# ivannz/cplxmodule

Measured on AMD Instinct MI355X. Metric: Cplx-samples/sec fwd+bwd (CplxLinear-4096 + VD), higher is better.
Workload: dtype bf16; 1 GPU; CplxLinearVD 4096->4096, bf16 activations / fp32 master weights, batch 8192 per GPU, LRT fwd + KL + full bwd (BASELINE configs[1] + VD); global_batch=8192, parallelism=dp1, noise=in-kernel Philox4x32-7, launch=hipGraph replay, warmup_detail=5 eager steps (capture prerequisites) + 5 untimed replays

## Files before the change

### cplxmodule_amd/csrc/gemm.h

```cpp
#pragma once
#include "common.h"
#include "launch.h"

namespace cplxamd {

struct GemmArgs {
  const void* a_r; const void* a_i; int64_t a_rs, a_cs;
  const void* b_r; const void* b_i; int64_t b_rs, b_cs;
  const float* bias_r; const float* bias_i; const float* emul;
  void* c_r; void* c_i; int64_t ldc;
  int M, N, K;
  int conj_b, accumulate;
  int order = 1, group_m = 4, lds_epilogue = 1;
  int splits = 1; int kchunk = 0; void* ws = nullptr; int64_t ws_bytes = 0;
  const float* g1 = nullptr; const float* g2 = nullptr; float gsign = 1.0f;
  int batch = 1; int64_t a_bs = 0, b_bs = 0, c_bs = 0;
  const float* beta = nullptr; int emul_exp = 0;
  int emul_both = 0;
  const void* fx_r = nullptr; const void* fx_i = nullptr; const void* fga = nullptr; int64_t fld = 0;
  const float* scale_a = nullptr; const float* scale_b = nullptr;
  int flags = 0;
  int* plan = nullptr; int ncu = 0;
};

__device__ __forceinline__ float gemm_beta(const GemmArgs& g) { return (g.accumulate && g.beta) ? *g.beta : 1.0f; }
__device__ __forceinline__ float gemm_alpha(const GemmArgs& g) { return g.scale_a ? g.scale_a[1] * g.scale_b[1] : 1.0f; }
__device__ __forceinline__ float gemm_alpha_inv(const GemmArgs& g) { return g.scale_a ? g.scale_a[0] * g.scale_b[0] : 1.0f; }

__device__ __forceinline__ float gemm_emul(const GemmArgs& g, float m) { return g.emul_exp ? expf(m) : m; }

template <bool CPLX>
int launch_gemm_generic(const GemmArgs& g, int in_dtype, int out_dtype, hipStream_t st);

int64_t gemm_generic_ws_bytes(int M, int N, int K, bool cplx);

template <bool CPLX>
int launch_gemm_bf16(const GemmArgs& g, int out_dtype, hipStream_t st);

int launch_gemm_bf16_w4(const GemmArgs& g, bool cplx, int out_dtype, bool ta, bool tb, hipStream_t st, bool& taken);

int launch_gemm_bf16_gauss(const GemmArgs& g, int out_dtype, hipStream_t st);
int64_t gemm_bf16_gauss_ws_bytes(int M, int N, int K);


int64_t gemm_bf16_ws_bytes(int M, int N, int K, bool cplx);

template <bool CPLX>
int launch_gemm_f16(const GemmArgs& g, int out_dtype, hipStream_t st);
int launch_gemm_f16_w4(const GemmArgs& g, bool cplx, int out_dtype, bool ta, bool tb, hipStream_t st, bool& taken);

}
```

### cplxmodule_amd/csrc/gemm_bf16_impl.h

```cpp
#include <type_traits>

#include "gemm.h"
#include "prims.h"

namespace cplxamd {

constexpr int BK = 32, STAGES = 3;
template <bool CPLX>
struct Cfg {
  static constexpr int NT = 512;
  static constexpr int IB = CPLX ? 2 : 4;
  static constexpr int JB = 2;
  static constexpr int WM = CPLX ? 4 : 2, WN = CPLX ? 2 : 4;
  static constexpr int BM = 32 * IB * WM, BN = 32 * JB * WN;
  static constexpr int A_BYTES = BM * BK * 2, B_BYTES = BN * BK * 2;
  static constexpr int STAGE_BYTES = (CPLX ? 2 : 1) * (A_BYTES + B_BYTES);
  static constexpr int SMEM = STAGES * STAGE_BYTES;
  static constexpr int PA = BM * 4 / NT, PB = BN * 4 / NT;
  static constexpr int LOADS = (CPLX ? 2 : 1) * (PA + PB);
};


template <int ROWS, bool T, int NT>
__device__ __forceinline__ uint32_t piece_voff(int64_t ld, int row0, int rows, int j) {
  const int p = j * NT + (int)threadIdx.x;
  if (!T) {
    const int row = p >> 2;
    const int kc = (p & 3) ^ ((row >> 2) & 3);
    int grow = row0 + row;
    grow = grow < rows ? grow : rows - 1;
    return (uint32_t)(((int64_t)(grow - row0) * ld + kc * 8) * 2);
  }
  constexpr int CPR = ROWS / 8;
  const int k = p / CPR;
  const int c = (p % CPR) ^ ((k & 3) << 2);
  int col = row0 + c * 8;
  col = col + 8 <= rows ? col : rows - 8;
  return (uint32_t)(((int64_t)k * ld + (col - row0)) * 2);
}
template <bool T>
__device__ __forceinline__ const bf16_t* piece_base(const bf16_t* plane, int64_t ld, int row0, int k0) {
  return T ? plane + (int64_t)k0 * ld + row0 : plane + (int64_t)row0 * ld + (int64_t)k0;
}

__device__ __forceinline__ bf16x8 frag_n(const char* lds_plane, int row, int kc) {
  const int off = row * 64 + ((kc ^ ((row >> 2) & 3)) << 4);
  return *reinterpret_cast<const bf16x8*>(lds_plane + off);
}

template <int ROWS>
__device__ __forceinline__ bf16x8 frag_t(const char* lds_plane, int rb, int kb, int m) {
  const int r = rb + 4 * (m & 3);
  s16x4 v[2];
#pragma unroll
  for (int h = 0; h < 2; ++h) {
    const int k = kb + 4 * h + (m >> 2);
    const int off = k * (ROWS * 2) + (((r >> 3) ^ ((k & 3) << 2)) << 4) + (r & 7) * 2;
    v[h] = __builtin_amdgcn_ds_read_tr16_b64_v4i16(
        (__attribute__((address_space(3))) s16x4*)(lds_plane + off));
  }
  const s16x8 both = __builtin_shufflevector(v[0], v[1], 0, 1, 2, 3, 4, 5, 6, 7);
  return __builtin_bit_cast(bf16x8, both);
}

__device__ __forceinline__ void nt_store16(void* p, uint4 v) { *reinterpret_cast<uint4*>(p) = v; }
__device__ __forceinline__ void nt_store16(float* p, const f4& a) { st4(p, a); }

template <typename TOUT, bool CPLX, bool CONJ, bool TA, bool TB>
__global__ __launch_bounds__((Cfg<CPLX>::NT), 2) void gemm_bf16_kernel(GemmArgs g) {
  extern __shared__ __attribute__((aligned(16))) char smem[];
  using C = Cfg<CPLX>;
  constexpr int NT = C::NT;

  constexpr int BM = C::BM, BN = C::BN, IB = C::IB, JB = C::JB;
  const int tiles_m = (g.M + BM - 1) / BM, tiles_n = (g.N + BN - 1) / BN;
  const int ntiles = tiles_m * tiles_n;
  int lin = blockIdx.x, split = 0;
  if (g.splits > 1) { split = lin / ntiles; lin -= split * ntiles; }
  int bm, bn;
  if (g.order == 0) {
    bm = lin / tiles_n; bn = lin - bm * tiles_n;
  } else {
    const int q = ntiles >> 3, r = ntiles & 7, xcd = lin & 7, idx = lin >> 3;
    lin = (xcd < r ? xcd * (q + 1) : r * (q + 1) + (xcd - r) * q) + idx;
    const int GM = g.group_m;
    const int per_group = GM * tiles_n;
    const int grp = lin / per_group, in_grp = lin - grp * per_group;
    const int first_m = grp * GM;
    const int gm = (tiles_m - first_m) < GM ? (tiles_m - first_m) : GM;
    bm = first_m + in_grp % gm; bn = in_grp / gm;
  }
  const int m0 = __builtin_amdgcn_readfirstlane(bm * BM), n0 = __builtin_amdgcn_readfirstlane(bn * BN);

  const int lane = threadIdx.x & 63, wid = threadIdx.x >> 6;
  const int wm = (wid / C::WN) * (32 * IB), wn = (wid % C::WN) * (32 * JB);
  const int l31 = lane & 31, lk = lane >> 5;
  const int l15 = lane & 15, lg = (lane >> 4) & 1;

  const bf16_t* Ar = (const bf16_t*)g.a_r; const bf16_t* Ai = (const bf16_t*)g.a_i;
  const bf16_t* Br = (const bf16_t*)g.b_r; const bf16_t* Bi = (const bf16_t*)g.b_i;
  const int64_t lda = TA ? g.a_cs : g.a_rs, ldb = TB ? g.b_cs : g.b_rs;

  f32x16 acc_r[IB][JB], acc_i[CPLX ? IB : 1][JB];
#pragma unroll
  for (int i = 0; i < IB; ++i)
#pragma unroll
    for (int j = 0; j < JB; ++j) {
      acc_r[i][j] = f32x16{0};
      if (CPLX) acc_i[i][j] = f32x16{0};
    }

  const bool bias_in_acc = g.bias_r != nullptr && g.g1 == nullptr && g.splits <= 1;
  f4 bias_v[CPLX ? 2 : 1][JB][4];
  if (bias_in_acc) {
    const bool vec = (g.N & 3) == 0 && (reinterpret_cast<uintptr_t>(g.bias_r) & 15) == 0 &&
                     (!CPLX || (reinterpret_cast<uintptr_t>(g.bias_i) & 15) == 0);
#pragma unroll
    for (int pl = 0; pl < (CPLX ? 2 : 1); ++pl) {
      const float* bias = pl ? g.bias_i : g.bias_r;
#pragma unroll
      for (int j = 0; j < JB; ++j)
#pragma unroll
        for (int q = 0; q < 4; ++q) {
          const int col = n0 + wn + j * 32 + 8 * q + 4 * lk;
          if (vec && col + 3 < g.N) {
            bias_v[pl][j][q] = ld4(bias + col);
          } else {
#pragma unroll
            for (int e = 0; e < 4; ++e) bias_v[pl][j][q].v[e] = col + e < g.N ? bias[col + e] : 0.f;
          }
        }
    }
#ifdef CPLXAMD_GEMM_F16
    if (g.scale_a) {
      const float inv = gemm_alpha_inv(g);
#pragma unroll
      for (int pl = 0; pl < (CPLX ? 2 : 1); ++pl)
#pragma unroll
        for (int j = 0; j < JB; ++j)
#pragma unroll
          for (int q = 0; q < 4; ++q)
#pragma unroll
            for (int e = 0; e < 4; ++e) bias_v[pl][j][q].v[e] *= inv;
    }
#endif
  }
  auto apply_bias = [&]() __attribute__((always_inline)) {
    if (!bias_in_acc) return;
#pragma unroll
    for (int i = 0; i < IB; ++i)
#pragma unroll
      for (int j = 0; j < JB; ++j)
#pragma unroll
        for (int q = 0; q < 4; ++q)
#pragma unroll
          for (int e = 0; e < 4; ++e) {
            acc_r[i][j][4 * q + e] = bias_v[0][j][q].v[e];
            if (CPLX) acc_i[i][j][4 * q + e] = bias_v[CPLX ? 1 : 0][j][q].v[e];
          }
  };
  const int kbase = __builtin_amdgcn_readfirstlane(split * g.kchunk);
  const uint32_t smem_off = lds_offset_of(smem);
  const uint32_t wave_lds = (uint32_t)__builtin_amdgcn_readfirstlane(threadIdx.x >> 6) * 1024u;
  uint32_t voa[C::PA], vob[C::PB];
#pragma unroll
  for (int j = 0; j < C::PA; ++j) voa[j] = piece_voff<BM, TA, NT>(lda, m0, g.M, j);
#pragma unroll
  for (int j = 0; j < C::PB; ++j) vob[j] = piece_voff<BN, TB, NT>(ldb, n0, g.N, j);
  auto stage_q = [&](int buf, int k0, int q) __attribute__((always_inline)) {
    k0 += kbase;
    const uint32_t s = smem_off + (uint32_t)(buf * C::STAGE_BYTES) + wave_lds;
    if (q < C::PA)
      lds_dma16_sv(piece_base<TA>(Ar, lda, m0, k0), voa[q], s + q * NT * 16);
    else if (q < C::PA + C::PB)
      lds_dma16_sv(piece_base<TB>(Br, ldb, n0, k0), vob[q - C::PA], s + C::A_BYTES + (q - C::PA) * NT * 16);
    else if (q < 2 * C::PA + C::PB)
      lds_dma16_sv(piece_base<TA>(Ai, lda, m0, k0), voa[q - C::PA - C::PB],
                   s + C::A_BYTES + C::B_BYTES + (q - C::PA - C::PB) * NT * 16);
    else
      lds_dma16_sv(piece_base<TB>(Bi, ldb, n0, k0), vob[q - 2 * C::PA - C::PB],
                   s + 2 * C::A_BYTES + C::B_BYTES + (q - 2 * C::PA - C::PB) * NT * 16);
  };
  auto stage_all = [&](int buf, int k0) __attribute__((always_inline)) {
#pragma unroll
    for (int q = 0; q < C::LOADS; ++q) stage_q(buf, k0, q);
  };

  auto a_frag = [&](const char* plane, int i, int ks) __attribute__((always_inline)) -> bf16x8 {
    if (TA) return frag_t<BM>(plane, wm + i * 32 + 16 * lg, ks * 16 + 8 * lk, l15);
    return frag_n(plane, wm + i * 32 + l31, ks * 2 + lk);
  };
  auto b_frag = [&](const char* plane, int j, int ks) __attribute__((always_inline)) -> bf16x8 {
    if (TB) return frag_t<BN>(plane, wn + j * 32 + 16 * lg, ks * 16 + 8 * lk, l15);
    return frag_n(plane, wn + j * 32 + l31, ks * 2 + lk);
  };

  const int klen = g.splits > 1 ? ((g.K - kbase) < g.kchunk ? (g.K - kbase) : g.kchunk) : g.K;
  const int nt = __builtin_amdgcn_readfirstlane(klen / BK);
  {
    bf16x8 ar[2][IB], br[2][JB], ai[2][IB], bi[2][JB];
    auto read_half = [&](int buf, int ks) __attribute__((always_inline)) {
      const char* sA = smem + buf * C::STAGE_BYTES;
      const char* sB = sA + C::A_BYTES;
      const char* sAi = sB + C::B_BYTES;
      const char* sBi = sAi + C::A_BYTES;
#pragma unroll
      for (int i = 0; i < IB; ++i) {
        ar[ks][i] = a_frag(sA, i, ks);
        if (CPLX) ai[ks][i] = a_frag(sAi, i, ks);
      }
#pragma unroll
      for (int j = 0; j < JB; ++j) {
        br[ks][j] = b_frag(sB, j, ks);
        if (CPLX) bi[ks][j] = b_frag(sBi, j, ks);
      }
    };
    constexpr int NFRAG = CPLX ? 2 * IB + 4 : IB + JB;
    auto read_one = [&](int buf, int ks, int idx) __attribute__((always_inline)) {
      const char* sA = smem + buf * C::STAGE_BYTES;
      const char* sB = sA + C::A_BYTES;
      const char* sAi = sB + C::B_BYTES;
      const char* sBi = sAi + C::A_BYTES;
      if (CPLX) {
        if (idx == 0) br[ks][0] = b_frag(sB, 0, ks);
        else if (idx == 1) bi[ks][0] = b_frag(sBi, 0, ks);
        else if (idx == 2) ar[ks][0] = a_frag(sA, 0, ks);
        else if (idx == 3) ai[ks][0] = a_frag(sAi, 0, ks);
        else if (idx == 4) br[ks][1] = b_frag(sB, 1, ks);
        else if (idx == 5) bi[ks][1] = b_frag(sBi, 1, ks);
        else if ((idx & 1) == 0) ar[ks][(idx - 4) / 2] = a_frag(sA, (idx - 4) / 2, ks);
        else ai[ks][(idx - 5) / 2] = a_frag(sAi, (idx - 5) / 2, ks);
      } else {
        if (idx == 0) br[ks][0] = b_frag(sB, 0, ks);
        else if (idx == 1) ar[ks][0] = a_frag(sA, 0, ks);
        else if (idx == 2) br[ks][1] = b_frag(sB, 1, ks);
        else if (idx == 3) ar[ks][1] = a_frag(sA, 1, ks);
        else if (idx < 2 + JB) br[ks][idx - 2] = b_frag(sB, idx - 2, ks);
        else ar[ks][idx - JB] = a_frag(sA, idx - JB, ks);
      }
    };
    constexpr int H = (C::LOADS + 1) / 2;
    auto mfma_half = [&](int ks, int slot, int tile, int q0, int q1, int rbuf, int rks) __attribute__((always_inline)) {
      bf16x8 nai[IB];
      if (CPLX) {
#pragma unroll
        for (int i = 0; i < IB; ++i) nai[i] = neg_frag(CONJ ? ar[ks][i] : ai[ks][i]);
      }
      int q = q0;
      const int k0s = (tile < nt ? tile : nt - 1) * BK;
      if constexpr (CPLX) {
        constexpr int NG = 2 * IB * JB;
#pragma unroll
        for (int ph = 0; ph < 2; ++ph)
#pragma unroll
          for (int i = 0; i < IB; ++i)
#pragma unroll
            for (int j = 0; j < JB; ++j) {
              if (ph == 0) {
                acc_r[i][j] = CPLXAMD_MFMA16(br[ks][j], ar[ks][i], acc_r[i][j]);
                acc_i[i][j] = CPLXAMD_MFMA16(br[ks][j], ai[ks][i], acc_i[i][j]);
              } else if (CONJ) {
                acc_r[i][j] = CPLXAMD_MFMA16(bi[ks][j], ai[ks][i], acc_r[i][j]);
                acc_i[i][j] = CPLXAMD_MFMA16(bi[ks][j], nai[i], acc_i[i][j]);
              } else {
                acc_r[i][j] = CPLXAMD_MFMA16(bi[ks][j], nai[i], acc_r[i][j]);
                acc_i[i][j] = CPLXAMD_MFMA16(bi[ks][j], ar[ks][i], acc_i[i][j]);
              }
              constexpr int PER = (NFRAG + NG - 1) / NG;
              const int g0 = (ph * IB * JB + i * JB + j) * PER;
              __builtin_amdgcn_sched_barrier(0);
#pragma unroll
              for (int r = 0; r < PER; ++r)
                if (g0 + r < NFRAG) read_one(rbuf, rks, g0 + r);
              __builtin_amdgcn_sched_barrier(0);
              if (q < q1) {
                __builtin_amdgcn_sched_barrier(0);
                stage_q(slot, k0s, q);
                __builtin_amdgcn_sched_barrier(0);
                ++q;
              }
            }
        return;
      }
#pragma unroll
      for (int i = 0; i < IB; ++i)
#pragma unroll
        for (int j = 0; j < JB; ++j) {
          acc_r[i][j] = CPLXAMD_MFMA16(br[ks][j], ar[ks][i], acc_r[i][j]);
          if (CPLX) {
            acc_i[i][j] = CPLXAMD_MFMA16(br[ks][j], ai[ks][i], acc_i[i][j]);
            if (CONJ) {
              acc_r[i][j] = CPLXAMD_MFMA16(bi[ks][j], ai[ks][i], acc_r[i][j]);
              acc_i[i][j] = CPLXAMD_MFMA16(bi[ks][j], nai[i], acc_i[i][j]);
            } else {
              acc_r[i][j] = CPLXAMD_MFMA16(bi[ks][j], nai[i], acc_r[i][j]);
              acc_i[i][j] = CPLXAMD_MFMA16(bi[ks][j], ar[ks][i], acc_i[i][j]);
            }
          }
          {
            constexpr int PER = (NFRAG + IB * JB - 1) / (IB * JB);
            const int g0 = (i * JB + j) * PER;
            __builtin_amdgcn_sched_barrier(0);
#pragma unroll
            for (int r = 0; r < PER; ++r)
              if (g0 + r < NFRAG) read_one(rbuf, rks, g0 + r);
            __builtin_amdgcn_sched_barrier(0);
          }
          if (q < q1) {
            __builtin_amdgcn_sched_barrier(0);
            stage_q(slot, k0s, q);
            __builtin_amdgcn_sched_barrier(0);
            ++q;
          }
        }
    };
    stage_all(0, 0);
    if (nt > 1) stage_all(1, BK);
    apply_bias();
    if (nt > 1) wait_vmcnt<C::LOADS>(); else wait_vmcnt<0>();
    __builtin_amdgcn_s_barrier();
    read_half(0, 0);
#pragma unroll
    for (int q = 0; q < H; ++q) stage_q(2, (nt > 2 ? 2 : nt - 1) * BK, q);
    auto tile_body = [&](int cur, int nx1, int nx2, int t) __attribute__((always_inline)) {
      mfma_half(0, nx2, t + 2, H, C::LOADS, cur, 1);
      asm volatile("s_waitcnt lgkmcnt(0)" ::: "memory");
      wait_vmcnt<C::LOADS>();
      __builtin_amdgcn_s_barrier();
      mfma_half(1, cur, t + 3, 0, H, nx1, 0);
    };
    int t = 0;
    for (; t + 3 <= nt; t += 3) {
      tile_body(0, 1, 2, t);
      tile_body(1, 2, 0, t + 1);
      tile_body(2, 0, 1, t + 2);
    }
    if (t < nt) tile_body(0, 1, 2, t);
    if (t + 1 < nt) tile_body(1, 2, 0, t + 1);
  }

#ifdef CPLXAMD_GEMM_F16
  if (g.scale_a) {
    const float alpha = gemm_alpha(g);
#pragma unroll
    for (int i = 0; i < IB; ++i)
#pragma unroll
      for (int j = 0; j < JB; ++j) {
        acc_r[i][j] *= alpha;
        if (CPLX) acc_i[i][j] *= alpha;
      }
  }
#endif

  TOUT* cr = reinterpret_cast<TOUT*>(g.c_r);
  TOUT* ci = reinterpret_cast<TOUT*>(g.c_i);
  const float beta = gemm_beta(g);
  if (g.splits > 1) {
    const int64_t slab = (int64_t)g.M * g.ldc;
    cr = reinterpret_cast<TOUT*>(g.ws) + (int64_t)split * (CPLX ? 2 : 1) * slab;
    ci = cr + slab;
  }
  if constexpr (sizeof(TOUT) == 2) {
    const bool lds_epi = JB == 2 && g.lds_epilogue && !g.g1 && !g.emul && !g.accumulate && g.splits <= 1 && (g.ldc & 7) == 0 &&
                         (reinterpret_cast<uintptr_t>(cr) & 15) == 0 &&
                         (!CPLX || (reinterpret_cast<uintptr_t>(ci) & 15) == 0);
    if (lds_epi) {
      constexpr int PITCH = 144;
      wait_vmcnt<0>();
      __syncthreads();
      char* reg = smem + wid * (64 * PITCH);
#pragma unroll
      for (int pl = 0; pl < (CPLX ? 2 : 1); ++pl) {
        TOUT* out = pl ? ci : cr;
        const float* bias = pl ? g.bias_i : g.bias_r;
#pragma unroll
        for (int ih = 0; ih < IB / 2; ++ih) {
#pragma unroll
          for (int ii = 0; ii < 2; ++ii)
#pragma unroll
            for (int j = 0; j < JB; ++j)
#pragma unroll
              for (int q = 0; q < 4; ++q) {
                const int cl = j * 32 + 8 * q + 4 * lk;
                const int col = n0 + wn + cl;
                f4 v;
#pragma unroll
                for (int e = 0; e < 4; ++e) {
                  const float b = (bias && !bias_in_acc && col + e < g.N) ? bias[col + e] : 0.f;
                  v.v[e] = (pl ? acc_i[CPLX ? ih * 2 + ii : 0][j][4 * q + e] : acc_r[ih * 2 + ii][j][4 * q + e]) + b;
                }
                st4(reinterpret_cast<bf16_t*>(reg + (ii * 32 + l31) * PITCH + cl * 2), v);
              }
          asm volatile("s_waitcnt lgkmcnt(0)" ::: "memory");
#pragma unroll
          for (int pass = 0; pass < 8; ++pass) {
            const int rl = pass * 8 + (lane >> 3), c8 = (lane & 7) * 8;
            const uint4 v = *reinterpret_cast<const uint4*>(reg + rl * PITCH + c8 * 2);
            const int row = m0 + wm + ih * 64 + rl, col = n0 + wn + c8;
            if (row < g.M && col < g.N) {
              bf16_t* o = reinterpret_cast<bf16_t*>(out) + (int64_t)row * g.ldc + col;
              if (col + 7 < g.N) {
                if (g.fga) {
                  const int64_t fo = (int64_t)row * g.fld + col;
                  const uint4 gv = *reinterpret_cast<const uint4*>(reinterpret_cast<const bf16_t*>(g.fga) + fo);
                  const uint4 xv = *reinterpret_cast<const uint4*>(reinterpret_cast<const bf16_t*>(pl ? g.fx_i : g.fx_r) + fo);
                  const uint32_t vw[4] = {v.x, v.y, v.z, v.w}, xw[4] = {xv.x, xv.y, xv.z, xv.w}, gw[4] = {gv.x, gv.y, gv.z, gv.w};
                  uint32_t ow[4];
#pragma unroll
                  for (int e = 0; e < 4; ++e) {
                    const float d0 = __uint_as_float(vw[e] << 16), d1 = __uint_as_float(vw[e] & 0xffff0000u);
                    const float x0 = __uint_as_float(xw[e] << 16), x1 = __uint_as_float(xw[e] & 0xffff0000u);
                    const float g0 = __uint_as_float(gw[e] << 16), g1 = __uint_as_float(gw[e] & 0xffff0000u);
                    ow[e] = pack_bf16(fmaf(2.0f * x0, g0, d0), fmaf(2.0f * x1, g1, d1));
                  }
                  nt_store16(o, uint4{ow[0], ow[1], ow[2], ow[3]});
                } else {
                  nt_store16(o, v);
                }
              } else {
                const uint32_t w4[4] = {v.x, v.y, v.z, v.w};
#pragma unroll
                for (int w = 0; w < 4; ++w) {
                  if (col + 2 * w < g.N) o[2 * w] = (bf16_t)(w4[w] & 0xffffu);
                  if (col + 2 * w + 1 < g.N) o[2 * w + 1] = (bf16_t)(w4[w] >> 16);
                }
              }
            }
          }
          asm volatile("s_waitcnt lgkmcnt(0)" ::: "memory");
        }
      }
      return;
    }
  }
  if constexpr (sizeof(TOUT) == 4) {
    const bool lds_epi = JB == 2 && g.lds_epilogue && !g.g1 && g.splits <= 1 && (g.ldc & 3) == 0 &&
                         (reinterpret_cast<uintptr_t>(cr) & 15) == 0 &&
                         (!CPLX || (reinterpret_cast<uintptr_t>(ci) & 15) == 0) &&
                         (!g.emul || (reinterpret_cast<uintptr_t>(g.emul) & 15) == 0);
    if (lds_epi) {
      constexpr int PITCH = 272;
      wait_vmcnt<0>();
      __syncthreads();
      char* reg = smem + wid * (32 * PITCH);
#pragma unroll
      for (int pl = 0; pl < (CPLX ? 2 : 1); ++pl) {
        float* out = reinterpret_cast<float*>(pl ? ci : cr);
        const float* bias = pl ? g.bias_i : g.bias_r;
#pragma unroll
        for (int i = 0; i < IB; ++i) {
#pragma unroll
          for (int j = 0; j < JB; ++j)
#pragma unroll
            for (int q = 0; q < 4; ++q) {
              const int cl = j * 32 + 8 * q + 4 * lk;
              const int col = n0 + wn + cl;
              f4 v;
#pragma unroll
              for (int e = 0; e < 4; ++e) {
                const float b = (bias && !bias_in_acc && col + e < g.N) ? bias[col + e] : 0.f;
                v.v[e] = (pl ? acc_i[CPLX ? i : 0][j][4 * q + e] : acc_r[i][j][4 * q + e]) + b;
              }
              st4(reinterpret_cast<float*>(reg + l31 * PITCH + cl * 4), v);
            }
          asm volatile("s_waitcnt lgkmcnt(0)" ::: "memory");
#pragma unroll
          for (int pass = 0; pass < 8; ++pass) {
            const int rl = pass * 4 + (lane >> 4), c4 = (lane & 15) * 4;
            f4 v = ld4(reinterpret_cast<const float*>(reg + rl * PITCH + c4 * 4));
            const int row = m0 + wm + i * 32 + rl, col = n0 + wn + c4;
            if (row < g.M && col < g.N) {
              const int64_t o = (int64_t)row * g.ldc + col;
              if (col + 3 < g.N) {
                if (g.emul && (!pl || g.emul_both)) {
                  const f4 m = ld4(g.emul + o);
#pragma unroll
                  for (int e = 0; e < 4; ++e) v.v[e] *= gemm_emul(g, m.v[e]);
                }
                if (g.accumulate) {
                  const f4 p = ld4(out + o);
#pragma unroll
                  for (int e = 0; e < 4; ++e) v.v[e] += beta * p.v[e];
                }
                nt_store16(out + o, v);
              } else {
#pragma unroll
                for (int e = 0; e < 4; ++e)
                  if (col + e < g.N) {
                    float x = v.v[e];
                    if (g.emul && (!pl || g.emul_both)) x *= gemm_emul(g, g.emul[o + e]);
                    if (g.accumulate) x += beta * out[o + e];
                    out[o + e] = x;
                  }
              }
            }
          }
          asm volatile("s_waitcnt lgkmcnt(0)" ::: "memory");
        }
      }
      return;
    }
  }
  const bool two_planes = CPLX || g.g1;
  const bool vec_ok = (g.ldc & 3) == 0 && (reinterpret_cast<uintptr_t>(cr) & 15) == 0 &&
                      (!two_planes || (reinterpret_cast<uintptr_t>(ci) & 15) == 0) &&
                      (!g.g1 || (g.N & 3) == 0) &&
                      (!g.emul || (reinterpret_cast<uintptr_t>(g.emul) & 15) == 0);
  auto store_block = [&](auto I) __attribute__((always_inline)) {
    constexpr int i = decltype(I)::value;
    const int row = m0 + wm + i * 32 + l31;
    if (row >= g.M) return;
#pragma unroll
    for (int j = 0; j < JB; ++j) {
#pragma unroll
      for (int q = 0; q < 4; ++q) {
        const int col = n0 + wn + j * 32 + 8 * q + 4 * lk;
        if (col >= g.N) continue;
        const int64_t o = (int64_t)row * g.ldc + col;
        f4 vr, vi;
#pragma unroll
        for (int e = 0; e < 4; ++e) {
          vr.v[e] = acc_r[i][j][4 * q + e];
          vi.v[e] = CPLX ? acc_i[CPLX ? i : 0][j][4 * q + e] : 0.f;
        }
        if (!CPLX && g.g1) {
          const int64_t od = (int64_t)row * g.N + col;
          if (vec_ok && col + 3 < g.N) {
            const f4 p = ld4(g.g1 + od), t2 = ld4(g.g2 + od);
#pragma unroll
            for (int e = 0; e < 4; ++e) {
              const float q = g.gsign * t2.v[e];
              vi.v[e] = vr.v[e] - p.v[e] - q;
              vr.v[e] = p.v[e] - q;
            }
            if (g.bias_r) {
              const f4 b = ld4(g.bias_r + col), c = ld4(g.bias_i + col);
#pragma unroll
              for (int e = 0; e < 4; ++e) { vr.v[e] += b.v[e]; vi.v[e] += c.v[e]; }
            }
            st4(cr + o, vr);
            st4(ci + o, vi);
          } else {
            for (int e = 0; e < 4 && col + e < g.N; ++e) {
              const float p = g.g1[od + e], q = g.gsign * g.g2[od + e];
              io<TOUT>::st(cr + o + e, p - q + (g.bias_r ? g.bias_r[col + e] : 0.f));
              io<TOUT>::st(ci + o + e, vr.v[e] - p - q + (g.bias_i ? g.bias_i[col + e] : 0.f));
            }
          }
          continue;
        }
        if (vec_ok && col + 3 < g.N) {
          if (g.bias_r && !bias_in_acc) {
            const f4 b = ld4(g.bias_r + col);
#pragma unroll
            for (int e = 0; e < 4; ++e) vr.v[e] += b.v[e];
            if (CPLX) {
              const f4 c = ld4(g.bias_i + col);
#pragma unroll
              for (int e = 0; e < 4; ++e) vi.v[e] += c.v[e];
            }
          }
          if (g.emul) {
            const f4 m = ld4(g.emul + o);
#pragma unroll
            for (int e = 0; e < 4; ++e) vr.v[e] *= gemm_emul(g, m.v[e]);
            if (CPLX && g.emul_both) {
#pragma unroll
              for (int e = 0; e < 4; ++e) vi.v[e] *= gemm_emul(g, m.v[e]);
            }
          }
          if (g.accumulate) {
            const f4 p = ld4(cr + o);
#pragma unroll
            for (int e = 0; e < 4; ++e) vr.v[e] += beta * p.v[e];
            if (CPLX) {
              const f4 p2 = ld4(ci + o);
#pragma unroll
              for (int e = 0; e < 4; ++e) vi.v[e] += beta * p2.v[e];
            }
          }
          st4(cr + o, vr);
          if (CPLX) st4(ci + o, vi);
        } else {
#pragma unroll
          for (int e = 0; e < 4; ++e) {
            if (col + e >= g.N) break;
            float xr = vr.v[e] + ((g.bias_r && !bias_in_acc) ? g.bias_r[col + e] : 0.f);
            if (g.emul) xr *= gemm_emul(g, g.emul[o + e]);
            if (g.accumulate) xr += beta * io<TOUT>::ld(cr + o + e);
            io<TOUT>::st(cr + o + e, xr);
            if (CPLX) {
              float xi = vi.v[e] + ((g.bias_i && !bias_in_acc) ? g.bias_i[col + e] : 0.f);
              if (g.emul && g.emul_both) xi *= gemm_emul(g, g.emul[o + e]);
              if (g.accumulate) xi += beta * io<TOUT>::ld(ci + o + e);
              io<TOUT>::st(ci + o + e, xi);
            }
          }
        }
      }
    }
  };
  store_block(std::integral_constant<int, 0>{});
  store_block(std::integral_constant<int, 1>{});
  if constexpr (IB == 4) {
    store_block(std::integral_constant<int, 2>{});
    store_block(std::integral_constant<int, 3>{});
  }
  wait_vmcnt<0>();
}

template <typename TOUT, bool CPLX, bool CONJ, bool TA, bool TB>
static int launch_kernel_r(const GemmArgs& g, hipStream_t st) {
  using C = Cfg<CPLX>;
  const int64_t tiles = (int64_t)((g.M + C::BM - 1) / C::BM) * ((g.N + C::BN - 1) / C::BN);
  if (tiles * g.splits > 0x7fffffff) return CPLXAMD_ESHAPE;
  if (g.plan) { *g.plan = 1; return 0; }
  static PerDeviceOnce attr_set;
  if (const int e = set_max_dyn_lds(attr_set, gemm_bf16_kernel<TOUT, CPLX, CONJ, TA, TB>, C::SMEM)) return e;
  gemm_bf16_kernel<TOUT, CPLX, CONJ, TA, TB><<<dim3((unsigned)(tiles * g.splits)), C::NT, C::SMEM, st>>>(g);
  CPLXAMD_CHECK_LAUNCH();
  return 0;
}

}
#include "gemm_bf16_persist.h"
namespace cplxamd {

template <typename TOUT, bool CPLX, bool CONJ, bool TA, bool TB>
static int launch_persist(const GemmArgs& g, hipStream_t st, bool& taken) {
  using C = Cfg<CPLX>;
  taken = false;
  if (!launch_owns_chip(g.flags)) return 0;
  const int ncu = (g.ncu > 0 ? g.ncu : device_cus()) & ~7;
  if (g.splits > 1 || g.g1 || g.emul || g.accumulate || g.scale_a || (g.M % C::BM) || (g.N % C::BN) || g.K / BK < 12) return 0;
  if (g.fga && (!((CPLX ? CONJ : true) && TB && !TA && sizeof(TOUT) == 2) || (g.fld & 7) || !aligned16(g.fga) ||
                !aligned16(g.fx_r) || (CPLX && !aligned16(g.fx_i)) || g.bias_r)) return 0;
  constexpr bool kBf16Out = sizeof(TOUT) == 2;
  constexpr bool kInstantiated = !TA && (CPLX ? (CONJ == TB && kBf16Out) : (kBf16Out || !TB));
  if (!kInstantiated) return 0;
  const int64_t tiles = (int64_t)(g.M / C::BM) * (g.N / C::BN);
  if (tiles <= ncu || tiles > 0x7fffffff) return 0;
  const int align = sizeof(TOUT) == 2 ? 7 : 3;
  if ((g.ldc & align) || !aligned16(g.c_r) || (CPLX && !aligned16(g.c_i))) return 0;
  if (g.bias_r && (!aligned16(g.bias_r) || (CPLX && !aligned16(g.bias_i)))) return 0;
  constexpr int smem = 3 * C::STAGE_BYTES + 16384;
  if constexpr (kInstantiated) {
    constexpr bool kFusable = (CPLX ? CONJ : true) && TB && kBf16Out;
    auto go = [&](auto RR) -> int {
      constexpr int R = decltype(RR)::value;
      if (g.plan) { *g.plan = 2; return 0; }
      if constexpr (kFusable) {
        if (g.fga) {
          static PerDeviceOnce attr_set_f;
          if (const int e = set_max_dyn_lds(attr_set_f, gemm_bf16_persist_kernel<TOUT, CPLX, CONJ, TA, TB, R, true>, smem)) return e;
          gemm_bf16_persist_kernel<TOUT, CPLX, CONJ, TA, TB, R, true><<<dim3((unsigned)ncu), C::NT, smem, st>>>(g);
          CPLXAMD_CHECK_LAUNCH();
          return 0;
        }
      }
      static PerDeviceOnce attr_set;
      if (const int e = set_max_dyn_lds(attr_set, gemm_bf16_persist_kernel<TOUT, CPLX, CONJ, TA, TB, R>, smem)) return e;
      gemm_bf16_persist_kernel<TOUT, CPLX, CONJ, TA, TB, R><<<dim3((unsigned)ncu), C::NT, smem, st>>>(g);
      CPLXAMD_CHECK_LAUNCH();
      return 0;
    };
    const int r = (g.K / BK) % 3;
    const int rc = r == 0 ? go(std::integral_constant<int, 0>{}) : r == 1 ? go(std::integral_constant<int, 1>{})
                                                                          : go(std::integral_constant<int, 2>{});
    if (rc) return rc;
    taken = true;
  }
  return 0;
}

template <typename TOUT, bool CPLX, bool CONJ, bool TA, bool TB>
static int launch_kernel(const GemmArgs& g, hipStream_t st) {
  {
    bool taken = false;
    const int rc = launch_gemm_bf16_w4(g, CPLX, sizeof(TOUT) == 2 ? CPLXAMD_BF16 : CPLXAMD_F32, TA, TB, st, taken);
    if (rc || taken) return rc;
  }
  {
    bool taken = false;
    const int rc = launch_persist<TOUT, CPLX, CONJ, TA, TB>(g, st, taken);
    if (rc || taken) return rc;
  }
  if (g.fga) {
    const bool ok = sizeof(TOUT) == 2 && Cfg<CPLX>::JB == 2 && g.lds_epilogue && !g.g1 && !g.emul && !g.accumulate && g.splits <= 1 &&
                    !g.bias_r && (g.ldc & 7) == 0 && (g.fld & 7) == 0 && (g.N & 7) == 0 && aligned16(g.c_r) &&
                    (!CPLX || aligned16(g.c_i)) && aligned16(g.fga) && aligned16(g.fx_r) && (!CPLX || aligned16(g.fx_i));
    if (!ok) return CPLXAMD_ESHAPE;
  }
  return launch_kernel_r<TOUT, CPLX, CONJ, TA, TB>(g, st);
}

template <typename TOUT, bool CPLX, bool CONJ>
static int launch_layout(const GemmArgs& g, bool ta, bool tb, hipStream_t st) {
  if (ta) return tb ? launch_kernel<TOUT, CPLX, CONJ, true, true>(g, st)
                    : launch_kernel<TOUT, CPLX, CONJ, true, false>(g, st);
  return tb ? launch_kernel<TOUT, CPLX, CONJ, false, true>(g, st)
            : launch_kernel<TOUT, CPLX, CONJ, false, false>(g, st);
}

template <bool CPLX>
static int launch_dtype(const GemmArgs& g, int out_dtype, bool ta, bool tb, hipStream_t st) {
  if (out_dtype != CPLXAMD_BF16 && out_dtype != CPLXAMD_F32) return CPLXAMD_EINVAL;
  const bool f32 = out_dtype == CPLXAMD_F32;
#ifdef CPLXAMD_GEMM_F16
  if (!f32) return CPLXAMD_ESHAPE;
  if constexpr (CPLX) {
    if (g.conj_b) return launch_layout<float, true, true>(g, ta, tb, st);
  }
  return launch_layout<float, CPLX, false>(g, ta, tb, st);
#else
  if constexpr (CPLX) {
    if (g.conj_b)
      return f32 ? launch_layout<float, true, true>(g, ta, tb, st)
                 : launch_layout<bf16_t, true, true>(g, ta, tb, st);
  }
  return f32 ? launch_layout<float, CPLX, false>(g, ta, tb, st)
             : launch_layout<bf16_t, CPLX, false>(g, ta, tb, st);
#endif
}

static int plan_splits(int M, int N, int K, bool cplx) {
  const int bm = cplx ? Cfg<true>::BM : Cfg<false>::BM, bn = cplx ? Cfg<true>::BN : Cfg<false>::BN;
  const int64_t tiles = (int64_t)((M + bm - 1) / bm) * ((N + bn - 1) / bn);
  if (tiles >= 192 || K < 64 * BK) return 1;
  int s = (int)(256 / tiles);
  const int maxs = K / (32 * BK);
  if (s > maxs) s = maxs;
  if (s > 16) s = 16;
  return s < 2 ? 1 : s;
}

#if GEMM_BF16_TU == 1 && !defined(CPLXAMD_GEMM_F16)
int64_t gemm_bf16_ws_bytes(int M, int N, int K, bool cplx) {
  const int s = plan_splits(M, N, K, cplx);
  return s > 1 ? (int64_t)s * (cplx ? 2 : 1) * M * N * (int64_t)sizeof(float) : 0;
}
#endif

static __global__ __launch_bounds__(256) void gemm_slab_reduce_kernel(const float* slabs, int splits,
                                                               int64_t slab_stride, int M, int N,
                                                               int64_t ldc, const float* bias,
                                                               const float* emul, int emul_exp, int accumulate,
                                                               const float* beta_p, float* out) {
  const float beta = (accumulate && beta_p) ? *beta_p : 1.0f;
  const int64_t n4 = ((int64_t)M * ldc) >> 2;
  const int64_t stride = (int64_t)gridDim.x * 256;
  for (int64_t i = (int64_t)blockIdx.x * 256 + threadIdx.x; i < n4; i += stride) {
    f4 acc = ld4(slabs + 4 * i);
    for (int s = 1; s < splits; ++s) {
      const f4 v = ld4(slabs + (int64_t)s * slab_stride + 4 * i);
#pragma unroll
      for (int e = 0; e < 4; ++e) acc.v[e] += v.v[e];
    }
    const int col = (int)((4 * i) % ldc);
#pragma unroll
    for (int e = 0; e < 4; ++e) {
      if (bias && col + e < N) acc.v[e] += bias[col + e];
    }
    if (emul) {
      const f4 m = ld4(emul + 4 * i);
#pragma unroll
      for (int e = 0; e < 4; ++e) acc.v[e] *= emul_exp ? expf(m.v[e]) : m.v[e];
    }
    if (accumulate) {
      const f4 o = ld4(out + 4 * i);
#pragma unroll
      for (int e = 0; e < 4; ++e) acc.v[e] += beta * o.v[e];
    }
    st4(out + 4 * i, acc);
  }
}

template <bool CPLX>
static int launch_splitk(const GemmArgs& g0, int splits, bool ta, bool tb, hipStream_t st) {
  GemmArgs g = g0;
  g.splits = splits;
  g.kchunk = ((g.K / BK + splits - 1) / splits) * BK;
  GemmArgs k = g;
  k.ldc = g.N; k.bias_r = k.bias_i = nullptr; k.emul = nullptr; k.accumulate = 0;
  const int rc = launch_dtype<CPLX>(k, CPLXAMD_F32, ta, tb, st);
  if (rc) return rc;
  if (g.plan) { *g.plan = *g.plan == 3 ? 5 : 4; return 0; }
  const int64_t slab = (int64_t)g.M * g.N, stride = (CPLX ? 2 : 1) * slab;
  const int grid = stream_grid(slab >> 2, 256);
  gemm_slab_reduce_kernel<<<grid, 256, 0, st>>>((const float*)g.ws, splits, stride, g.M, g.N, g.ldc,
                                                g.bias_r, g.emul, g.emul_exp, g.accumulate, g.beta, (float*)g.c_r);
  CPLXAMD_CHECK_LAUNCH();
  if (CPLX) {
    gemm_slab_reduce_kernel<<<grid, 256, 0, st>>>((const float*)g.ws + slab, splits, stride, g.M, g.N,
                                                  g.ldc, g.bias_i, g.emul_both ? g.emul : nullptr, g.emul_exp, g.accumulate, g.beta,
                                                  (float*)g.c_i);
    CPLXAMD_CHECK_LAUNCH();
  }
  return 0;
}

template <bool CPLX>
int launch_gemm_bf16(const GemmArgs& g, int out_dtype, hipStream_t st) {
  bool ta, tb;
  if (g.a_cs == 1) ta = false; else if (g.a_rs == 1) ta = true; else return CPLXAMD_ESHAPE;
  if (g.b_cs == 1) tb = false; else if (g.b_rs == 1) tb = true; else return CPLXAMD_ESHAPE;
  if (g.K < BK || (g.K % BK) != 0) return CPLXAMD_ESHAPE;
  const int64_t lda = ta ? g.a_cs : g.a_rs, ldb = tb ? g.b_cs : g.b_rs;
  if ((lda % 8) != 0 || (ldb % 8) != 0) return CPLXAMD_ESHAPE;
  if (lda >= (1 << 22) || ldb >= (1 << 22)) return CPLXAMD_ESHAPE;
  if ((ta && ((g.M % 8) != 0 || g.M < 8)) || (tb && ((g.N % 8) != 0 || g.N < 8))) return CPLXAMD_ESHAPE;
  if (!aligned16(g.a_r) || !aligned16(g.b_r)) return CPLXAMD_ESHAPE;
  if (CPLX && (!aligned16(g.a_i) || !aligned16(g.b_i))) return CPLXAMD_ESHAPE;
  if (g.M <= 0 || g.N <= 0) return 0;
  if (out_dtype == CPLXAMD_F32 && g.ws && g.ldc == g.N && (g.N & 3) == 0) {
    const int splits = plan_splits(g.M, g.N, g.K, CPLX);
    if (splits > 1 && g.ws_bytes >= gemm_bf16_ws_bytes(g.M, g.N, g.K, CPLX))
      return launch_splitk<CPLX>(g, splits, ta, tb, st);
  }
  return launch_dtype<CPLX>(g, out_dtype, ta, tb, st);
}

#if GEMM_BF16_TU == 1 && !defined(CPLXAMD_GEMM_F16)
__global__ __launch_bounds__(256) void gauss_sum_kernel(const bf16_t* r, const bf16_t* i, float sign,
                                                        bf16_t* out, int64_t n8) {
  const int64_t stride = (int64_t)gridDim.x * 256;
  for (int64_t c = (int64_t)blockIdx.x * 256 + threadIdx.x; c < n8; c += stride) {
    const uint4 a = *reinterpret_cast<const uint4*>(r + 8 * c);
    const uint4 b = *reinterpret_cast<const uint4*>(i + 8 * c);
    const uint32_t aw[4] = {a.x, a.y, a.z, a.w}, bw[4] = {b.x, b.y, b.z, b.w};
    uint32_t ow[4];
#pragma unroll
    for (int e = 0; e < 4; ++e) {
      const float lo = __uint_as_float(aw[e] << 16) + sign * __uint_as_float(bw[e] << 16);
      const float hi = __uint_as_float(aw[e] & 0xffff0000u) + sign * __uint_as_float(bw[e] & 0xffff0000u);
      ow[e] = pack_bf16(lo, hi);
    }
    *reinterpret_cast<uint4*>(out + 8 * c) = uint4{ow[0], ow[1], ow[2], ow[3]};
  }
}

static int64_t align256(int64_t x) { return (x + 255) & ~(int64_t)255; }

int64_t gemm_bf16_gauss_ws_bytes(int M, int N, int K) {
  return align256((int64_t)M * K * 2) + align256((int64_t)N * K * 2) + 2 * (int64_t)M * N * 4;
}

int launch_gemm_bf16_gauss(const GemmArgs& g, int out_dtype, hipStream_t st) {
  bool ta, tb;
  if (g.a_cs == 1) ta = false; else if (g.a_rs == 1) ta = true; else return CPLXAMD_ESHAPE;
  if (g.b_cs == 1) tb = false; else if (g.b_rs == 1) tb = true; else return CPLXAMD_ESHAPE;
  if ((ta ? g.a_cs : g.a_rs) != (ta ? g.M : g.K) || (tb ? g.b_cs : g.b_rs) != (tb ? g.N : g.K))
    return CPLXAMD_ESHAPE;
  if (g.accumulate || (g.N & 3) || ((int64_t)g.M * g.K & 7) || ((int64_t)g.N * g.K & 7))
    return CPLXAMD_ESHAPE;
  if (!g.ws || g.ws_bytes < gemm_bf16_gauss_ws_bytes(g.M, g.N, g.K)) return CPLXAMD_EWS;
  if ((reinterpret_cast<uintptr_t>(g.ws) & 255) != 0) return CPLXAMD_EALIGN;
  if (g.M <= 0 || g.N <= 0) return 0;
  char* w = (char*)g.ws;
  bf16_t* As = (bf16_t*)w; w += align256((int64_t)g.M * g.K * 2);
  bf16_t* Bs = (bf16_t*)w; w += align256((int64_t)g.N * g.K * 2);
  float* t1 = (float*)w; float* t2 = t1 + (int64_t)g.M * g.N;
  const float s = g.conj_b ? -1.0f : 1.0f;
  const int64_t na = (int64_t)g.M * g.K / 8, nb = (int64_t)g.N * g.K / 8;
  gauss_sum_kernel<<<stream_grid(na, 256), 256, 0, st>>>((const bf16_t*)g.a_r, (const bf16_t*)g.a_i,
                                                        1.0f, As, na);
  CPLXAMD_CHECK_LAUNCH();
  gauss_sum_kernel<<<stream_grid(nb, 256), 256, 0, st>>>((const bf16_t*)g.b_r, (const bf16_t*)g.b_i,
                                                        s, Bs, nb);
  CPLXAMD_CHECK_LAUNCH();
  GemmArgs r = g;
  r.a_i = r.b_i = nullptr; r.bias_r = r.bias_i = nullptr; r.conj_b = 0;
  r.ws = nullptr; r.ws_bytes = 0; r.ldc = g.N; r.c_i = nullptr;
  r.c_r = t1;
  int rc = launch_gemm_bf16<false>(r, CPLXAMD_F32, st);
  if (rc) return rc;
  r.a_r = g.a_i; r.b_r = g.b_i; r.c_r = t2;
  rc = launch_gemm_bf16<false>(r, CPLXAMD_F32, st);
  if (rc) return rc;
  GemmArgs f = g;
  f.a_r = As; f.b_r = Bs; f.a_i = f.b_i = nullptr; f.conj_b = 0; f.ws = nullptr; f.ws_bytes = 0;
  f.g1 = t1; f.g2 = t2; f.gsign = s;
  return launch_gemm_bf16<false>(f, out_dtype, st);
}
#endif

#if GEMM_BF16_TU == 1
template int launch_gemm_bf16<false>(const GemmArgs&, int, hipStream_t);
#else
template int launch_gemm_bf16<true>(const GemmArgs&, int, hipStream_t);
#endif

}
```

### cplxmodule_amd/csrc/gemm_bf16_w4.hip

```cpp
#include <type_traits>

#include "gemm.h"
#include "prims.h"

namespace cplxamd {
namespace w4 {

typedef uint32_t u32x4 __attribute__((ext_vector_type(4)));

constexpr int BK = 32;

template <bool CPLX>
struct Cfg {
  static constexpr int NT = 256;
  static constexpr int IB = 4, JB = CPLX ? 2 : 4;
  static constexpr int WM = 2, WN = 2;
  static constexpr int BM = 32 * IB * WM, BN = 32 * JB * WN;
  static constexpr int NPL = CPLX ? 2 : 1;
  static constexpr int A_BYTES = BM * BK * 2, B_BYTES = BN * BK * 2;
  static constexpr int SLOT = NPL * (A_BYTES + B_BYTES);
  static constexpr int SMEM = 3 * SLOT;
  static constexpr int PA = BM * 4 / NT, PB = BN * 4 / NT;
  static constexpr int NL = NPL * (PA + PB);
  static constexpr int NFRAG = NPL * (IB + JB);
  static constexpr int NM = NPL * NPL * IB * JB;
};

template <int ROWS, bool T>
__device__ __forceinline__ uint32_t src_voff(int64_t ld, int tid) {
  if (!T) return (uint32_t)((((int64_t)(tid >> 2)) * ld + (tid & 3) * 8) * 2);
  constexpr int CPR = ROWS / 8;
  return (uint32_t)((((int64_t)(tid / CPR)) * ld + (tid % CPR) * 8) * 2);
}
template <int ROWS, bool T>
__device__ __forceinline__ uint32_t piece_stride(int64_t ld) {
  constexpr int NT = 256;
  if (!T) return (uint32_t)((NT / 4) * ld * 2);
  return (uint32_t)((NT / (ROWS / 8)) * ld * 2);
}
template <int ROWS, bool T>
__device__ __forceinline__ uint32_t dst_off(int tid) {
  if (!T) {
    const int row = tid >> 2, c = tid & 3;
    return (uint32_t)(row * 64 + ((c ^ ((row >> 2) & 3)) << 4));
  }
  constexpr int CPR = ROWS / 8;
  const int k = tid / CPR, c = tid % CPR;
  return (uint32_t)(k * (ROWS * 2) + ((c ^ ((k & 3) << 2)) << 4));
}

typedef __attribute__((address_space(3))) const bf16x8* lds_frag_p;
typedef __attribute__((address_space(3))) s16x4* lds_tr_p;
typedef __attribute__((address_space(3))) u32x4* lds_st_p;
__device__ __forceinline__ bf16x8 lds_frag_n(uint32_t addr, int imm) { return *(lds_frag_p)(uintptr_t)(addr + (uint32_t)imm); }
template <int ROWS>
__device__ __forceinline__ bf16x8 lds_frag_t(uint32_t addr, int imm) {
  const s16x4 v0 = __builtin_amdgcn_ds_read_tr16_b64_v4i16((lds_tr_p)(uintptr_t)(addr + (uint32_t)imm));
  const s16x4 v1 = __builtin_amdgcn_ds_read_tr16_b64_v4i16((lds_tr_p)(uintptr_t)(addr + (uint32_t)(imm + 4 * ROWS * 2)));
  const s16x8 both = __builtin_shufflevector(v0, v1, 0, 1, 2, 3, 4, 5, 6, 7);
  return __builtin_bit_cast(bf16x8, both);
}
__device__ __forceinline__ uint32_t lane_n(int worg, int lane, int ks) {
  const int row = worg + (lane & 31), kc = ks * 2 + (lane >> 5);
  return (uint32_t)(row * 64 + ((kc ^ ((row >> 2) & 3)) << 4));
}
template <int ROWS>
__device__ __forceinline__ uint32_t lane_t(int worg, int lane, int blk) {
  const int m = lane & 15, k = 8 * (lane >> 5) + (m >> 2);
  const int r = worg + blk * 32 + 16 * ((lane >> 4) & 1) + 4 * (m & 3);
  return (uint32_t)(k * (ROWS * 2) + (((r >> 3) ^ ((k & 3) << 2)) << 4) + (r & 7) * 2);
}
__device__ __forceinline__ uint32_t opaque(uint32_t x) { asm volatile("" : "+v"(x)); return x; }
__device__ __forceinline__ void store16(void* p, uint4 v) {
  *reinterpret_cast<uint4*>(p) = v;
}
__device__ __forceinline__ void store16(float* p, const f4& a) {
  st4(p, a);
}

#define W4_SB() __builtin_amdgcn_sched_barrier(0)
#define W4_VMCNT(N) __builtin_amdgcn_s_waitcnt(0x0F70 | ((N) & 0xF) | ((((N) >> 4) & 3) << 14))

constexpr int write_slot(bool cplx, int k) { return cplx ? 6 + 4 * k : (k == 0 ? 6 : k == 1 ? 9 : k == 2 ? 11 : 14); }
constexpr int slot_of_write(bool cplx, int nw, int m) {
  for (int k = 0; k < nw; ++k)
    if (write_slot(cplx, k) == m) return k;
  return -1;
}

template <typename TOUT, bool CPLX, bool CONJ, bool TA, bool TB, bool PERSIST = false>
__device__ __forceinline__ void w4_tile(const GemmArgs& g, const int lin0, char* smem) {
  using C = Cfg<CPLX>;
  constexpr int NT = C::NT, BM = C::BM, BN = C::BN, IB = C::IB, JB = C::JB, NPL = C::NPL;
  constexpr int PA = C::PA, PB = C::PB, NL = C::NL, NFRAG = C::NFRAG, NM = C::NM, SLOT = C::SLOT;

  const int tiles_m = g.M / BM, tiles_n = g.N / BN;
  const int ntiles = tiles_m * tiles_n;
  int split = 0;
  auto origin = [&](int lin, int& om, int& on) __attribute__((always_inline)) {
    if (g.splits > 1) { split = lin / ntiles; lin -= split * ntiles; }
    const int q = ntiles >> 3, r = ntiles & 7, xcd = lin & 7, idx = lin >> 3;
    lin = (xcd < r ? xcd * (q + 1) : r * (q + 1) + (xcd - r) * q) + idx;
    const int GM = g.group_m;
    const int per_group = GM * tiles_n;
    const int grp = lin / per_group, in_grp = lin - grp * per_group;
    const int first_m = grp * GM;
    const int gm = (tiles_m - first_m) < GM ? (tiles_m - first_m) : GM;
    om = __builtin_amdgcn_readfirstlane((first_m + in_grp % gm) * BM);
    on = __builtin_amdgcn_readfirstlane((in_grp / gm) * BN);
  };
  int m0, n0;
  origin(lin0, m0, n0);

  const int tid = threadIdx.x;
  const int lane = tid & 63, wid = tid >> 6;
  const int wm = (wid / C::WN) * (32 * IB), wn = (wid % C::WN) * (32 * JB);
  const int l31 = lane & 31, lk = lane >> 5;
  const int l15 = lane & 15, lg = (lane >> 4) & 1;

  const int64_t lda = TA ? g.a_cs : g.a_rs, ldb = TB ? g.b_cs : g.b_rs;
  const int64_t ka = TA ? lda * 2 : 2, kb = TB ? ldb * 2 : 2;
  const char* pa[NPL]; const char* pb[NPL];
  auto plane_bases = [&](int tm, int tn, const char* (&qa)[NPL], const char* (&qb)[NPL]) __attribute__((always_inline)) {
    qa[0] = (const char*)g.a_r + (TA ? (int64_t)tm : (int64_t)tm * lda) * 2;
    qb[0] = (const char*)g.b_r + (TB ? (int64_t)tn : (int64_t)tn * ldb) * 2;
    if (CPLX) {
      qa[NPL - 1] = (const char*)g.a_i + (TA ? (int64_t)tm : (int64_t)tm * lda) * 2;
      qb[NPL - 1] = (const char*)g.b_i + (TB ? (int64_t)tn : (int64_t)tn * ldb) * 2;
    }
  };
  plane_bases(m0, n0, pa, pb);
  const char* pan[NPL]; const char* pbn[NPL]; const char* rqa[NPL]; const char* rqb[NPL];
  const int ntp = __builtin_amdgcn_readfirstlane(g.K / BK);
  auto set_request = [&](int kt, auto REDIR) __attribute__((always_inline)) {
    const bool nx = decltype(REDIR)::value && kt >= ntp;
    const int kk = (nx ? kt - ntp : kt) & ~1;
#pragma unroll
    for (int pl = 0; pl < NPL; ++pl) {
      rqa[pl] = (nx ? pan[pl] : pa[pl]) + (int64_t)kk * BK * ka;
      rqb[pl] = (nx ? pbn[pl] : pb[pl]) + (int64_t)kk * BK * kb;
    }
  };
  const int kbase = __builtin_amdgcn_readfirstlane(split * g.kchunk);
  if (g.splits > 1) {
#pragma unroll
    for (int pl = 0; pl < NPL; ++pl) { pa[pl] += (int64_t)kbase * ka; pb[pl] += (int64_t)kbase * kb; }
  }
  const uint32_t voa = src_voff<BM, TA>(lda, tid), vob = src_voff<BN, TB>(ldb, tid);
  const uint32_t psa = (uint32_t)__builtin_amdgcn_readfirstlane((int)piece_stride<BM, TA>(lda));
  const uint32_t psb = (uint32_t)__builtin_amdgcn_readfirstlane((int)piece_stride<BN, TB>(ldb));
  const uint32_t qa = TA ? (uint32_t)__builtin_amdgcn_readfirstlane((int)(uint32_t)(32 * ka)) : 0u;
  const uint32_t qb = TB ? (uint32_t)__builtin_amdgcn_readfirstlane((int)(uint32_t)(32 * kb)) : 0u;
  const uint32_t wra = dst_off<BM, TA>(tid), wrb = dst_off<BN, TB>(tid);

  f32x16 acc_r[IB][JB], acc_i[CPLX ? IB : 1][JB];

  const bool has_bias = g.bias_r != nullptr;
  f4 bias_v[NPL][JB][4];
  if (has_bias) {
#pragma unroll
    for (int pl = 0; pl < NPL; ++pl) {
      const float* bias = pl ? g.bias_i : g.bias_r;
#pragma unroll
      for (int j = 0; j < JB; ++j)
#pragma unroll
        for (int q = 0; q < 4; ++q) bias_v[pl][j][q] = ld4(bias + n0 + wn + j * 32 + 8 * q + 4 * lk);
    }
#ifdef CPLXAMD_GEMM_F16
    if (g.scale_a) {
      const float inv = gemm_alpha_inv(g);
#pragma unroll
      for (int pl = 0; pl < NPL; ++pl)
#pragma unroll
        for (int j = 0; j < JB; ++j)
#pragma unroll
          for (int q = 0; q < 4; ++q)
#pragma unroll
            for (int e = 0; e < 4; ++e) bias_v[pl][j][q].v[e] *= inv;
    }
#endif
  }

  u32x4 st[2][NL];
  auto load_piece = [&](auto PAR, auto Q, int kt) __attribute__((always_inline)) {
    constexpr int par = decltype(PAR)::value, q = decltype(Q)::value;
    constexpr int pl = q / (PA + PB), r = q % (PA + PB);
    constexpr bool isa = r < PA;
    constexpr int j = isa ? r : r - PA;
    const char* base;
    if constexpr (PERSIST) {
      base = isa ? rqa[pl] : rqb[pl];
    } else {
      const int64_t kby = (int64_t)(kt & ~1) * BK * (isa ? ka : kb);
      base = (isa ? pa[pl] : pb[pl]) + kby;
    }
    __amdgpu_buffer_rsrc_t rs = __builtin_amdgcn_make_buffer_rsrc((void*)base, 0, 0x7ffffffe, 0x00020000);
    const uint32_t so = (uint32_t)j * (isa ? psa : psb) + (par ? (isa ? qa : qb) : 0u);
    const uint32_t vo = (isa ? voa : vob) + ((par && !(isa ? TA : TB)) ? 64u : 0u);
    st[par][q] = __builtin_amdgcn_raw_buffer_load_b128(rs, vo, so, 0);
  };
  const uint32_t smem_off = (uint32_t)(uintptr_t)smem;
  uint32_t wa[3], wb[3];
  uint32_t sl[3];
#pragma unroll
  for (int s3 = 0; s3 < 3; ++s3) {
    wa[s3] = opaque(smem_off + s3 * SLOT + wra);
    wb[s3] = opaque(smem_off + s3 * SLOT + C::A_BYTES + wrb);
    sl[s3] = (uint32_t)(s3 * SLOT);
  }
  auto write_piece = [&](auto PAR, auto Q, auto WS) __attribute__((always_inline)) {
    constexpr int par = decltype(PAR)::value, q = decltype(Q)::value, ws = decltype(WS)::value;
    constexpr int pl = q / (PA + PB), r = q % (PA + PB);
    constexpr bool isa = r < PA;
    constexpr int j = isa ? r : r - PA;
    const uint32_t addr = (isa ? wa[ws] : wb[ws]) + (uint32_t)(pl * (C::A_BYTES + C::B_BYTES) + j * 4096);
    *(lds_st_p)(uintptr_t)(addr) = st[par][q];
  };
  constexpr int NFA = TA ? IB : 2, NFB = TB ? JB : 2;
  uint32_t fa[3][NFA], fb[3][NFB];
#pragma unroll
  for (int s3 = 0; s3 < 3; ++s3) {
#pragma unroll
    for (int x = 0; x < NFA; ++x)
      fa[s3][x] = opaque(smem_off + s3 * SLOT + (TA ? lane_t<BM>(wm, lane, x) : lane_n(wm, lane, x)));
#pragma unroll
    for (int x = 0; x < NFB; ++x)
      fb[s3][x] = opaque(smem_off + s3 * SLOT + C::A_BYTES + (TB ? lane_t<BN>(wn, lane, x) : lane_n(wn, lane, x)));
  }
  auto a_frag = [&](auto S, auto PL, auto BLK, auto KS) __attribute__((always_inline)) -> bf16x8 {
    constexpr int s3 = decltype(S)::value, pl = decltype(PL)::value, blk = decltype(BLK)::value, ks = decltype(KS)::value;
    constexpr int po = pl * (C::A_BYTES + C::B_BYTES);
    if constexpr (TA) return lds_frag_t<BM>(fa[s3][blk], po + ks * 16 * (BM * 2));
    else return lds_frag_n(fa[s3][ks], po + blk * 2048);
  };
  auto b_frag = [&](auto S, auto PL, auto BLK, auto KS) __attribute__((always_inline)) -> bf16x8 {
    constexpr int s3 = decltype(S)::value, pl = decltype(PL)::value, blk = decltype(BLK)::value, ks = decltype(KS)::value;
    constexpr int po = pl * (C::A_BYTES + C::B_BYTES);
    if constexpr (TB) return lds_frag_t<BN>(fb[s3][blk], po + ks * 16 * (BN * 2));
    else return lds_frag_n(fb[s3][ks], po + blk * 2048);
  };

  bf16x8 ar[IB + 1], ai[CPLX ? IB + 1 : 1], br[2][JB], bi[2][CPLX ? JB : 1], nbi[CPLX ? JB : 1];
  using PL0 = std::integral_constant<int, 0>; using PL1 = std::integral_constant<int, NPL - 1>;
  auto rd_a = [&](auto F, auto I, auto S, auto KS) __attribute__((always_inline)) {
    constexpr int f = decltype(F)::value, i = decltype(I)::value;
    constexpr int d = i < IB - 1 ? i : IB - 1 + f;
    ar[d] = a_frag(S, PL0{}, I, KS);
  };
  auto rd_ai = [&](auto F, auto I, auto S, auto KS) __attribute__((always_inline)) {
    constexpr int f = decltype(F)::value, i = decltype(I)::value;
    constexpr int d = i < IB - 1 ? i : IB - 1 + f;
    if constexpr (CPLX) ai[d] = a_frag(S, PL1{}, I, KS);
  };
  auto rd_b = [&](auto F, auto J, auto S, auto KS) __attribute__((always_inline)) {
    constexpr int f = decltype(F)::value;
    br[f][decltype(J)::value] = b_frag(S, PL0{}, J, KS);
  };
  auto rd_bi = [&](auto F, auto J, auto S, auto KS) __attribute__((always_inline)) {
    constexpr int f = decltype(F)::value;
    if constexpr (CPLX) bi[f][decltype(J)::value] = b_frag(S, PL1{}, J, KS);
  };

  auto mfma = [&](auto F, auto MM) __attribute__((always_inline)) {
    constexpr int f = decltype(F)::value, m = decltype(MM)::value;
    if constexpr (CPLX) {
      constexpr int i = m / 8, ph = (m % 8) / 4, j = (m % 4) / 2, c = m % 2;
      constexpr int d = i < IB - 1 ? i : IB - 1 + f;
      if constexpr (ph == 0) {
        if constexpr (c == 0) acc_r[i][j] = CPLXAMD_MFMA16(br[f][j], ar[d], acc_r[i][j]);
        else acc_i[i][j] = CPLXAMD_MFMA16(br[f][j], ai[d], acc_i[i][j]);
      } else if constexpr (CONJ) {
        if constexpr (c == 0) acc_r[i][j] = CPLXAMD_MFMA16(bi[f][j], ai[d], acc_r[i][j]);
        else acc_i[i][j] = CPLXAMD_MFMA16(nbi[j], ar[d], acc_i[i][j]);
      } else {
        if constexpr (c == 0) acc_r[i][j] = CPLXAMD_MFMA16(nbi[j], ai[d], acc_r[i][j]);
        else acc_i[i][j] = CPLXAMD_MFMA16(bi[f][j], ar[d], acc_i[i][j]);
      }
    } else {
      constexpr int i = m / JB, j = m % JB;
      constexpr int d = i < IB - 1 ? i : IB - 1 + f;
      acc_r[i][j] = CPLXAMD_MFMA16(br[f][j], ar[d], acc_r[i][j]);
    }
  };

  const int klen = g.splits > 1 ? ((g.K - kbase) < g.kchunk ? (g.K - kbase) : g.kchunk) : g.K;
  const int nt = __builtin_amdgcn_readfirstlane(klen / BK);

  auto sub = [&](auto F, auto PAR, auto H, auto RS, auto RKS, auto WS, int kt_next) __attribute__((always_inline)) {
    constexpr int f = decltype(F)::value, par = decltype(PAR)::value, h = decltype(H)::value;
    using I_F = std::integral_constant<int, f>;
    using I_G = std::integral_constant<int, 1 - f>;
    using I_P = std::integral_constant<int, par>;
    using I0_ = std::integral_constant<int, 0>; using I1_ = std::integral_constant<int, 1>;
    constexpr int G = NM / IB;
    constexpr int NW = NL / 2;
    auto slot_fill = [&](auto MM) __attribute__((always_inline)) {
      constexpr int m = decltype(MM)::value;
      if constexpr (m < NPL * JB) {
        if constexpr (CPLX) {
          if constexpr ((m & 1) == 0) rd_b(I_G{}, std::integral_constant<int, m / 2>{}, RS, RKS);
          else rd_bi(I_G{}, std::integral_constant<int, m / 2>{}, RS, RKS);
        } else {
          rd_b(I_G{}, std::integral_constant<int, m>{}, RS, RKS);
        }
      }
      if constexpr (CPLX && m < JB) nbi[m] = neg_frag(bi[f][m]);
      if constexpr (m == NPL * JB) rd_a(I_G{}, std::integral_constant<int, IB - 1>{}, RS, RKS);
      if constexpr (CPLX && m == NPL * JB + 1) rd_ai(I_G{}, std::integral_constant<int, IB - 1>{}, RS, RKS);
      if constexpr (m >= G && m % G == 0 && m / G <= IB - 1) rd_a(I_G{}, std::integral_constant<int, m / G - 1>{}, RS, RKS);
      if constexpr (CPLX && m >= G && m % G == 1 && m / G <= IB - 1) rd_ai(I_G{}, std::integral_constant<int, m / G - 1>{}, RS, RKS);
      constexpr int wi = slot_of_write(CPLX, NW, m);
      if constexpr (wi >= 0) {
        using PIECE = std::integral_constant<int, h * NW + wi>;
        write_piece(I_P{}, PIECE{}, WS);
        if constexpr (par == 1) {
          W4_SB(); load_piece(I0_{}, PIECE{}, kt_next);
          W4_SB(); load_piece(I1_{}, PIECE{}, kt_next);
        }
      }
    };
    auto run = [&](auto self, auto MM) __attribute__((always_inline)) {
      constexpr int m = decltype(MM)::value;
      if constexpr (m < NM) {
        mfma(I_F{}, MM);
        W4_SB();
        slot_fill(MM);
        W4_SB();
        self(self, std::integral_constant<int, m + 1>{});
      }
    };
    run(run, std::integral_constant<int, 0>{});
  };

  using I0 = std::integral_constant<int, 0>; using I1 = std::integral_constant<int, 1>; using I2 = std::integral_constant<int, 2>;
  auto for_pieces = [&](auto fn) __attribute__((always_inline)) {
    auto go = [&](auto self, auto Q) __attribute__((always_inline)) {
      constexpr int q = decltype(Q)::value;
      if constexpr (q < NL) { fn(Q); self(self, std::integral_constant<int, q + 1>{}); }
    };
    go(go, I0{});
  };
  int lin = lin0, mn = m0, nn = n0;
  bool has_next = false;
  auto look_ahead = [&]() __attribute__((always_inline)) {
    has_next = lin + (int)gridDim.x < ntiles;
    mn = m0; nn = n0;
    if (has_next) origin(lin + (int)gridDim.x, mn, nn);
    plane_bases(mn, nn, pan, pbn);
  };
  if constexpr (PERSIST) { look_ahead(); set_request(0, std::false_type{}); }
  for_pieces([&](auto Q) __attribute__((always_inline)) { load_piece(I0{}, Q, 0); load_piece(I1{}, Q, 0); });
#pragma unroll
  for (int i = 0; i < IB; ++i)
#pragma unroll
    for (int j = 0; j < JB; ++j)
#pragma unroll
      for (int q = 0; q < 4; ++q)
#pragma unroll
        for (int e = 0; e < 4; ++e) {
          acc_r[i][j][4 * q + e] = has_bias ? bias_v[0][j][q].v[e] : 0.f;
          if (CPLX) acc_i[i][j][4 * q + e] = has_bias ? bias_v[NPL - 1][j][q].v[e] : 0.f;
        }
  for_pieces([&](auto Q) __attribute__((always_inline)) {
    write_piece(I0{}, Q, I0{});
    write_piece(I1{}, Q, I1{});
  });
  {
    const int kt = nt > 2 ? 2 : nt - 2;
    if constexpr (PERSIST) set_request(kt, std::true_type{});
    for_pieces([&](auto Q) __attribute__((always_inline)) { load_piece(I0{}, Q, kt); load_piece(I1{}, Q, kt); });
  }
  asm volatile("s_waitcnt lgkmcnt(0)" ::: "memory");
  __builtin_amdgcn_s_barrier();
  auto first_frags = [&]() __attribute__((always_inline)) {
    auto goa = [&](auto self, auto I) __attribute__((always_inline)) {
      constexpr int i = decltype(I)::value;
      if constexpr (i < IB) { rd_a(I0{}, I, I0{}, I0{}); rd_ai(I0{}, I, I0{}, I0{}); self(self, std::integral_constant<int, i + 1>{}); }
    };
    auto gob = [&](auto self, auto J) __attribute__((always_inline)) {
      constexpr int j = decltype(J)::value;
      if constexpr (j < JB) { rd_b(I0{}, J, I0{}, I0{}); rd_bi(I0{}, J, I0{}, I0{}); self(self, std::integral_constant<int, j + 1>{}); }
    };
    gob(gob, I0{});
    goa(goa, I0{});
  };
  first_frags();

  auto tile = [&](auto SS, auto PP, int t, auto REDIR) __attribute__((always_inline)) {
    constexpr int s = decltype(SS)::value, par = decltype(PP)::value;
    using CUR = std::integral_constant<int, s>; using NXT = std::integral_constant<int, (s + 1) % 3>;
    using WR = std::integral_constant<int, (s + 2) % 3>;
    constexpr int ahead = 3;
    int ktn = (t + ahead < nt) ? t + ahead : nt - 2;
    if constexpr (PERSIST) {
      ktn = t + ahead;
      if constexpr (par == 1) set_request(ktn, REDIR);
    }
    sub(I0{}, PP, I0{}, CUR{}, I1{}, WR{}, ktn);
    asm volatile("s_waitcnt lgkmcnt(1)" ::: "memory");
    __builtin_amdgcn_s_barrier();
    W4_SB();
    sub(I1{}, PP, I1{}, NXT{}, I0{}, WR{}, ktn);
  };
  auto rotate = [&](auto R) __attribute__((always_inline)) {
    constexpr int r = decltype(R)::value;
    auto rot3 = [&](uint32_t& x0, uint32_t& x1, uint32_t& x2) __attribute__((always_inline)) {
      const uint32_t a = x0, b = x1, c = x2;
      if constexpr (r == 1) { x0 = b; x1 = c; x2 = a; } else { x0 = c; x1 = a; x2 = b; }
    };
    rot3(wa[0], wa[1], wa[2]); rot3(wb[0], wb[1], wb[2]); rot3(sl[0], sl[1], sl[2]);
#pragma unroll
    for (int x = 0; x < NFA; ++x) rot3(fa[0][x], fa[1][x], fa[2][x]);
#pragma unroll
    for (int x = 0; x < NFB; ++x) rot3(fb[0][x], fb[1][x], fb[2][x]);
  };
  do {
  {
    int t = 0;
    using RD = std::true_type;
    for (; t + 6 <= nt; t += 6) {
      tile(I0{}, I0{}, t, RD{});
      tile(I1{}, I1{}, t + 1, RD{});
      tile(I2{}, I0{}, t + 2, RD{});
      tile(I0{}, I1{}, t + 3, RD{});
      tile(I1{}, I0{}, t + 4, RD{});
      tile(I2{}, I1{}, t + 5, RD{});
    }
    if (t < nt) {
      tile(I0{}, I0{}, t, RD{});
      tile(I1{}, I1{}, t + 1, RD{});
      t += 2;
      if (t < nt) {
        tile(I2{}, I0{}, t, RD{});
        tile(I0{}, I1{}, t + 1, RD{});
        if constexpr (PERSIST) rotate(I1{});
      } else {
        if constexpr (PERSIST) rotate(I2{});
      }
    }
  }

#ifdef CPLXAMD_GEMM_F16
  if constexpr (!PERSIST) {
    if (g.scale_a) {
      const float alpha = gemm_alpha(g);
#pragma unroll
      for (int i = 0; i < IB; ++i)
#pragma unroll
        for (int j = 0; j < JB; ++j) {
          acc_r[i][j] *= alpha;
          if (CPLX) acc_i[i][j] *= alpha;
        }
    }
  }
#endif

  void* out_r = g.c_r;
  void* out_i = g.c_i;
  if (g.splits > 1) {
    const int64_t slab = (int64_t)g.M * g.ldc;
    float* base = reinterpret_cast<float*>(g.ws) + (int64_t)split * NPL * slab;
    out_r = base; out_i = base + slab;
  }
  const float beta = gemm_beta(g);
  asm volatile("s_waitcnt lgkmcnt(0)" ::: "memory");
  if constexpr (!PERSIST) __builtin_amdgcn_s_barrier();
  auto tile_rsrc = [&](const void* plane, int64_t ld, int esize) __attribute__((always_inline)) {
    const char* base = (const char*)plane + ((int64_t)m0 * ld + n0) * esize;
    return __builtin_amdgcn_make_buffer_rsrc((void*)base, 0, 0x7ffffffe, 0x00020000);
  };
  auto ldb128 = [](__amdgpu_buffer_rsrc_t r, uint32_t vo, uint32_t so) __attribute__((always_inline)) -> u32x4 {
    return __builtin_amdgcn_raw_buffer_load_b128(r, vo, so, 0);
  };
  auto stb128 = [](u32x4 v, __amdgpu_buffer_rsrc_t r, uint32_t vo, uint32_t so) __attribute__((always_inline)) {
    __builtin_amdgcn_raw_buffer_store_b128(v, r, vo, so, 0);
  };
  if constexpr (sizeof(TOUT) == 2) {
    auto epi16 = [&](auto FUSE) __attribute__((always_inline)) {
      constexpr bool fuse = decltype(FUSE)::value;
      constexpr int PITCH = 144;
      const int tid_e = PERSIST ? (int)opaque((uint32_t)tid) : tid;
      const int lane = tid_e & 63, wid = tid_e >> 6;
      const int wm = (wid / C::WN) * (32 * IB), wn = (wid % C::WN) * (32 * JB);
      const int l31 = lane & 31, lk = lane >> 5;
      const uint32_t vo_c = (uint32_t)((((int64_t)(wm + (lane >> 3)) * g.ldc + wn + (lane & 7) * 8)) * 2);
      char* reg = smem + (PERSIST ? (CPLX ? sl[2] : (uint32_t)C::SMEM) : 0u) + wid * (64 * PITCH);
      const uint32_t vo_f = fuse ? (uint32_t)((((int64_t)(wm + (lane >> 3)) * g.fld + wn + (lane & 7) * 8)) * 2) : 0u;
      const uint32_t p8c = (uint32_t)__builtin_amdgcn_readfirstlane((int)(uint32_t)(8 * g.ldc * 2));
      const uint32_t p8f = (uint32_t)__builtin_amdgcn_readfirstlane((int)(uint32_t)(8 * g.fld * 2));
      const __amdgpu_buffer_rsrc_t rga = tile_rsrc(fuse ? g.fga : g.c_r, fuse ? g.fld : g.ldc, 2);
      const __amdgpu_buffer_rsrc_t rout0 = tile_rsrc(out_r, g.ldc, 2), rout1 = tile_rsrc(CPLX ? out_i : out_r, g.ldc, 2);
      const __amdgpu_buffer_rsrc_t rx0 = tile_rsrc(fuse ? g.fx_r : g.c_r, fuse ? g.fld : g.ldc, 2);
      const __amdgpu_buffer_rsrc_t rx1 = tile_rsrc(fuse ? (CPLX ? g.fx_i : g.fx_r) : g.c_r, fuse ? g.fld : g.ldc, 2);
      constexpr int NR = NPL * (JB / 2) * (IB / 2);
      u32x4 gv[2][fuse ? 8 : 1], xv[2][fuse ? 8 : 1];
      auto load_ops = [&](int r) __attribute__((always_inline)) {
        const int pl = r / ((JB / 2) * (IB / 2)), jh = (r / (IB / 2)) % (JB / 2), ih = r % (IB / 2);
#pragma unroll
        for (int pass = 0; pass < 8; ++pass) {
          const uint32_t so = (uint32_t)(ih * 8 + pass) * p8f + (uint32_t)(jh * 128);
          gv[r & 1][pass] = ldb128(rga, vo_f, so);
          xv[r & 1][pass] = ldb128(pl ? rx1 : rx0, vo_f, so);
        }
      };
      if constexpr (fuse) load_ops(0);
      if constexpr (PERSIST) W4_VMCNT(0);
#pragma unroll
      for (int r = 0; r < NR; ++r) {
        const int pl = r / ((JB / 2) * (IB / 2)), jh = (r / (IB / 2)) % (JB / 2), ih = r % (IB / 2);
        const __amdgpu_buffer_rsrc_t rout = pl ? rout1 : rout0;
#pragma unroll
        for (int ii = 0; ii < 2; ++ii)
#pragma unroll
          for (int jj = 0; jj < 2; ++jj)
#pragma unroll
            for (int q = 0; q < 4; ++q) {
              const int cl = jj * 32 + 8 * q + 4 * lk;
              f4 v;
#pragma unroll
              for (int e = 0; e < 4; ++e) {
                const float a = pl ? acc_i[CPLX ? ih * 2 + ii : 0][jh * 2 + jj][4 * q + e] : acc_r[ih * 2 + ii][jh * 2 + jj][4 * q + e];
                v.v[e] = a;
              }
              st4(reinterpret_cast<bf16_t*>(reg + (ii * 32 + l31) * PITCH + cl * 2), v);
              if constexpr (PERSIST) W4_SB();
            }
        asm volatile("s_waitcnt lgkmcnt(0)" ::: "memory");
        if constexpr (fuse) {
          if (r + 1 < NR) { W4_SB(); load_ops(r + 1); W4_SB(); }
        }
#pragma unroll
        for (int pass = 0; pass < 8; ++pass) {
          const int rl = pass * 8 + (lane >> 3), c8 = (lane & 7) * 8;
          const u32x4 v = *reinterpret_cast<const u32x4*>(reg + rl * PITCH + c8 * 2);
          const uint32_t so = (uint32_t)(ih * 8 + pass) * p8c + (uint32_t)(jh * 128);
          if constexpr (fuse) {
            u32x4 ow;
#pragma unroll
            for (int e = 0; e < 4; ++e) {
              const float d0 = __uint_as_float(v[e] << 16), d1 = __uint_as_float(v[e] & 0xffff0000u);
              const float x0 = __uint_as_float(xv[r & 1][pass][e] << 16), x1 = __uint_as_float(xv[r & 1][pass][e] & 0xffff0000u);
              const float g0 = __uint_as_float(gv[r & 1][pass][e] << 16), g1 = __uint_as_float(gv[r & 1][pass][e] & 0xffff0000u);
              ow[e] = pack_bf16(fmaf(2.0f * x0, g0, d0), fmaf(2.0f * x1, g1, d1));
            }
            stb128(ow, rout, vo_c, so);
          } else {
            stb128(v, rout, vo_c, so);
          }
        }
        asm volatile("s_waitcnt lgkmcnt(0)" ::: "memory");
        if constexpr (PERSIST) W4_VMCNT(16);
        W4_SB();
      }
    };
    if constexpr (PERSIST) epi16(std::false_type{});
    else { if (g.fga) epi16(std::true_type{}); else epi16(std::false_type{}); }
  } else {
    auto epi32 = [&](auto HM, auto HACC) __attribute__((always_inline)) {
      constexpr bool hm = decltype(HM)::value, hacc = decltype(HACC)::value;
      constexpr int PITCH = 272;
      char* reg = smem + wid * (32 * PITCH);
      const uint32_t vo = (uint32_t)((((int64_t)(wm + (lane >> 4)) * g.ldc + wn + (lane & 15) * 4)) * 4);
      const uint32_t p4 = (uint32_t)__builtin_amdgcn_readfirstlane((int)(uint32_t)(4 * g.ldc * 4));
      const __amdgpu_buffer_rsrc_t rm = tile_rsrc(hm ? (const void*)g.emul : g.c_r, g.ldc, 4);
      const __amdgpu_buffer_rsrc_t rout0 = tile_rsrc(out_r, g.ldc, 4), rout1 = tile_rsrc(CPLX ? out_i : out_r, g.ldc, 4);
      constexpr int NR = NPL * (JB / 2) * IB;
      u32x4 mv[2][hm ? 8 : 1], pv[2][hacc ? 8 : 1];
      auto load_ops = [&](int r) __attribute__((always_inline)) {
        const int pl = r / ((JB / 2) * IB), jh = (r / IB) % (JB / 2), i = r % IB;
#pragma unroll
        for (int pass = 0; pass < 8; ++pass) {
          const uint32_t so = (uint32_t)(i * 8 + pass) * p4 + (uint32_t)(jh * 256);
          if constexpr (hm) mv[r & 1][pass] = ldb128(rm, vo, so);
          if constexpr (hacc) pv[r & 1][pass] = ldb128(pl ? rout1 : rout0, vo, so);
        }
      };
      if constexpr (hm || hacc) load_ops(0);
#pragma unroll
      for (int r = 0; r < NR; ++r) {
        const int pl = r / ((JB / 2) * IB), jh = (r / IB) % (JB / 2), i = r % IB;
        const __amdgpu_buffer_rsrc_t rout = pl ? rout1 : rout0;
#pragma unroll
        for (int jj = 0; jj < 2; ++jj)
#pragma unroll
          for (int q = 0; q < 4; ++q) {
            const int cl = jj * 32 + 8 * q + 4 * lk;
            f4 v;
#pragma unroll
            for (int e = 0; e < 4; ++e)
              v.v[e] = pl ? acc_i[CPLX ? i : 0][jh * 2 + jj][4 * q + e] : acc_r[i][jh * 2 + jj][4 * q + e];
            st4(reinterpret_cast<float*>(reg + l31 * PITCH + cl * 4), v);
          }
        asm volatile("s_waitcnt lgkmcnt(0)" ::: "memory");
        if constexpr (hm || hacc) {
          if (r + 1 < NR) { W4_SB(); load_ops(r + 1); W4_SB(); }
        }
#pragma unroll
        for (int pass = 0; pass < 8; ++pass) {
          const int rl = pass * 4 + (lane >> 4), c4 = (lane & 15) * 4;
          f4 v = ld4(reinterpret_cast<const float*>(reg + rl * PITCH + c4 * 4));
          const uint32_t so = (uint32_t)(i * 8 + pass) * p4 + (uint32_t)(jh * 256);
          if constexpr (hm) {
#pragma unroll
            for (int e = 0; e < 4; ++e) {
              v.v[e] *= gemm_emul(g, __uint_as_float(mv[r & 1][pass][e]));
              asm volatile("" : "+v"(v.v[e]));
            }
          }
          if constexpr (hacc) {
#pragma unroll
            for (int e = 0; e < 4; ++e) v.v[e] += beta * __uint_as_float(pv[r & 1][pass][e]);
          }
          const u32x4 w = {__float_as_uint(v.v[0]), __float_as_uint(v.v[1]), __float_as_uint(v.v[2]), __float_as_uint(v.v[3])};
          stb128(w, rout, vo, so);
        }
        asm volatile("s_waitcnt lgkmcnt(0)" ::: "memory");
        W4_SB();
      }
    };
    if (g.emul) { if (g.accumulate) epi32(std::true_type{}, std::true_type{}); else epi32(std::true_type{}, std::false_type{}); }
    else { if (g.accumulate) epi32(std::false_type{}, std::true_type{}); else epi32(std::false_type{}, std::false_type{}); }
  }
  if constexpr (!PERSIST) {
    break;
  } else {
    if (!has_next) break;
    __builtin_amdgcn_s_barrier();
    lin += (int)gridDim.x; m0 = mn; n0 = nn;
#pragma unroll
    for (int pl = 0; pl < NPL; ++pl) { pa[pl] = pan[pl]; pb[pl] = pbn[pl]; }
    look_ahead();
#pragma unroll
    for (int i = 0; i < IB; ++i)
#pragma unroll
      for (int j = 0; j < JB; ++j)
#pragma unroll
        for (int e = 0; e < 16; ++e) {
          acc_r[i][j][e] = 0.f;
          if (CPLX) acc_i[i][j][e] = 0.f;
        }
    first_frags();
    if constexpr (CPLX) {
      set_request(2, std::false_type{});
      for_pieces([&](auto Q) __attribute__((always_inline)) { load_piece(I0{}, Q, 2); load_piece(I1{}, Q, 2); });
    }
    if constexpr (!CPLX) W4_VMCNT(0);
  }
  } while (true);
}

template <typename TOUT, bool CPLX, bool CONJ, bool TA, bool TB>
__global__ __launch_bounds__(256) void gemm_bf16_w4_kernel(GemmArgs g) {
  extern __shared__ __attribute__((aligned(16))) char smem[];
  w4_tile<TOUT, CPLX, CONJ, TA, TB>(g, (int)blockIdx.x, smem);
}

template <bool CPLX, bool CONJ, bool TB>
__global__ __launch_bounds__(256) void gemm_bf16_w4p_kernel(GemmArgs g) {
  extern __shared__ __attribute__((aligned(16))) char smem[];
  w4_tile<bf16_t, CPLX, CONJ, false, TB, true>(g, (int)blockIdx.x, smem);
}

template <typename TOUT, bool CPLX, bool CONJ, bool TA, bool TB>
static int launch(const GemmArgs& g0, hipStream_t st) {
  using C = Cfg<CPLX>;
  GemmArgs g = g0;
  const int64_t tiles = (int64_t)(g.M / C::BM) * (g.N / C::BN);
  if constexpr (sizeof(TOUT) == 2 && !TA && !CPLX) {
    const int ncu = (g.ncu > 0 ? g.ncu : device_cus()) & ~7;
    const bool measured_faster = !CPLX && (!TB || g.K >= 4096);
    if (((launch_family(g.flags) >> 7) & 1) && measured_faster && launch_owns_chip(g.flags) && tiles > ncu && !g.fga &&
        !g.bias_r && g.splits <= 1) {
      if (g.plan) { *g.plan = 6; return 0; }
      static PerDeviceOnce attr_p;
      constexpr int smem_p = C::SMEM + (CPLX ? 0 : 4 * 64 * 144);
      if (const int e = set_max_dyn_lds(attr_p, gemm_bf16_w4p_kernel<CPLX, CONJ, TB>, smem_p)) return e;
      gemm_bf16_w4p_kernel<CPLX, CONJ, TB><<<dim3((unsigned)ncu), C::NT, smem_p, st>>>(g);
      CPLXAMD_CHECK_LAUNCH();
      return 0;
    }
  }
  if (g.plan) { *g.plan = 3; return 0; }
  static PerDeviceOnce attr_set;
  if (const int e = set_max_dyn_lds(attr_set, gemm_bf16_w4_kernel<TOUT, CPLX, CONJ, TA, TB>, C::SMEM)) return e;
  const int64_t grid = tiles * g.splits;
  gemm_bf16_w4_kernel<TOUT, CPLX, CONJ, TA, TB><<<dim3((unsigned)grid), C::NT, C::SMEM, st>>>(g);
  CPLXAMD_CHECK_LAUNCH();
  return 0;
}

template <typename TOUT, bool CPLX, bool CONJ>
static int launch_layout(const GemmArgs& g, bool ta, bool tb, hipStream_t st) {
  if (ta) return tb ? launch<TOUT, CPLX, CONJ, true, true>(g, st) : CPLXAMD_ESHAPE;
  return tb ? launch<TOUT, CPLX, CONJ, false, true>(g, st) : launch<TOUT, CPLX, CONJ, false, false>(g, st);
}

}

int launch_gemm_bf16_w4(const GemmArgs& g, bool cplx, int out_dtype, bool ta, bool tb, hipStream_t st, bool& taken) {
  taken = false;
  {
    const bool f32o = out_dtype == CPLXAMD_F32;
    const int bit = cplx ? (f32o ? 2 : g.fga ? 1 : 0) : (f32o ? 5 : g.fga ? 4 : 3);
    const int family = launch_family(g.flags);
    if (!((family >> bit) & 1)) return 0;
    if (!((family >> 6) & 1)) {
      const int keff = g.splits > 1 ? g.kchunk : g.K;
      if (keff < 1024) return 0;
      if (keff < 4096 && (ta || tb || g.fga)) return 0;
    }
  }
  const int bm = 256, bn = cplx ? 128 : 256;
  if (g.g1 || g.batch != 1) return 0;
  if (g.splits > 1) {
    const int last = g.K - (g.splits - 1) * g.kchunk;
    if (out_dtype != CPLXAMD_F32 || !g.ws || (g.kchunk % 64) || last < 128 || (last % 64) || g.kchunk < 128) return 0;
    if (g.bias_r || g.emul || g.accumulate || g.fga) return 0;
    if (!cplx) return 0;
  }
  if (ta && !tb) return 0;
  if ((g.M % bm) || (g.N % bn) || (g.K % 64) || g.K < 128) return 0;
  if ((int64_t)(g.M / bm) * (g.N / bn) * g.splits > 0x7fffffff) return 0;
  const int64_t lda = ta ? g.a_cs : g.a_rs, ldb = tb ? g.b_cs : g.b_rs;
  if ((lda % 8) || (ldb % 8) || lda >= (1 << 22) || ldb >= (1 << 22)) return 0;
  if (g.ldc >= (1 << 20) || g.fld >= (1 << 20)) return 0;
  if (!aligned16(g.a_r) || !aligned16(g.b_r) || !aligned16(g.c_r)) return 0;
  if (cplx && (!aligned16(g.a_i) || !aligned16(g.b_i) || !aligned16(g.c_i))) return 0;
  if (g.bias_r && (!aligned16(g.bias_r) || (cplx && !aligned16(g.bias_i)))) return 0;
  if (out_dtype == CPLXAMD_BF16) {
    if ((g.ldc & 7) || g.emul || g.accumulate) return 0;
    if (g.fga && ((g.fld & 7) || !aligned16(g.fga) || !aligned16(g.fx_r) || (cplx && !aligned16(g.fx_i)) || g.bias_r))
      return 0;
  } else if (out_dtype == CPLXAMD_F32) {
    if ((g.ldc & 3) || g.fga || (g.emul && !aligned16(g.emul))) return 0;
    if (cplx && g.emul && !g.emul_both) return 0;
  } else {
    return 0;
  }
  int rc;
  const bool f32 = out_dtype == CPLXAMD_F32;
#ifdef CPLXAMD_GEMM_F16
  if (!f32) return 0;
  if (cplx) rc = g.conj_b ? w4::launch_layout<float, true, true>(g, ta, tb, st) : w4::launch_layout<float, true, false>(g, ta, tb, st);
  else rc = w4::launch_layout<float, false, false>(g, ta, tb, st);
#else
  if (cplx) {
    if (g.conj_b) rc = f32 ? w4::launch_layout<float, true, true>(g, ta, tb, st) : w4::launch_layout<bf16_t, true, true>(g, ta, tb, st);
    else rc = f32 ? w4::launch_layout<float, true, false>(g, ta, tb, st) : w4::launch_layout<bf16_t, true, false>(g, ta, tb, st);
  } else {
    rc = f32 ? w4::launch_layout<float, false, false>(g, ta, tb, st) : w4::launch_layout<bf16_t, false, false>(g, ta, tb, st);
  }
#endif
  if (rc == CPLXAMD_ESHAPE) return 0;
  if (rc) return rc;
  taken = true;
  return 0;
}

}
```

### cplxmodule_amd/csrc/gemm_generic.hip

```cpp
#include "gemm.h"
#include "prims.h"

namespace cplxamd {


constexpr int GBK = 16;
template <int NB> struct GT {
  static constexpr int BM = 64 * NB, LD = BM + 1, PLANE = GBK * LD, PER = BM * GBK / 256;
};

template <typename T>
__device__ __forceinline__ float ldg(const void* p, int64_t off) {
  return io<T>::ld(reinterpret_cast<const T*>(p) + off);
}

template <int NB> struct TileRegs { float v[GT<NB>::PER]; };

template <typename TIN, int NB>
__device__ __forceinline__ TileRegs<NB> fetch_tile(const void* src, int64_t rs, int64_t cs, int row0,
                                               int k0, int rows, int K) {
  constexpr int BM = GT<NB>::BM, PER = GT<NB>::PER, KSTEP = 256 / BM;
  const int t = threadIdx.x;
  TileRegs<NB> o;
  if (cs == 1 || rs != 1) {
    const int k = t & 15, rb = t >> 4;
#pragma unroll
    for (int j = 0; j < PER; ++j) {
      const int gr = row0 + rb + 16 * j, gk = k0 + k;
      o.v[j] = (gr < rows && gk < K) ? ldg<TIN>(src, (int64_t)gr * rs + (int64_t)gk * cs) : 0.0f;
    }
  } else {
    const int r = t % BM, kb = t / BM;
#pragma unroll
    for (int j = 0; j < PER; ++j) {
      const int gr = row0 + r, gk = k0 + kb + KSTEP * j;
      o.v[j] = (gr < rows && gk < K) ? ldg<TIN>(src, (int64_t)gr * rs + (int64_t)gk * cs) : 0.0f;
    }
  }
  return o;
}

template <int NB>
__device__ __forceinline__ void commit_tile(float* dst, const TileRegs<NB>& o, int64_t rs, int64_t cs) {
  constexpr int BM = GT<NB>::BM, PER = GT<NB>::PER, KSTEP = 256 / BM, LD = GT<NB>::LD;
  const int t = threadIdx.x;
  if (cs == 1 || rs != 1) {
    const int k = t & 15, rb = t >> 4;
#pragma unroll
    for (int j = 0; j < PER; ++j) dst[k * LD + rb + 16 * j] = o.v[j];
  } else {
    const int r = t % BM, kb = t / BM;
#pragma unroll
    for (int j = 0; j < PER; ++j) dst[(kb + KSTEP * j) * LD + r] = o.v[j];
  }
}

template <typename TIN, typename TOUT, bool CPLX, int NB>
__global__ __launch_bounds__(256, 2) void gemm_generic_kernel(GemmArgs g) {
  extern __shared__ __attribute__((aligned(16))) float gsm[];
  constexpr int NPL = CPLX ? 4 : 2;
  constexpr int GBM = GT<NB>::BM, GBN = GT<NB>::BM, GLD = GT<NB>::LD, GPLANE = GT<NB>::PLANE;
  auto plane = [&](int buf, int which) { return gsm + (buf * NPL + which) * GPLANE; };

  const int m0 = blockIdx.y * GBM, n0 = blockIdx.x * GBN;
  const int lane = threadIdx.x & 63, wid = threadIdx.x >> 6;
  const int wm = (wid >> 1) * 32 * NB, wn = (wid & 1) * 32 * NB;
  const int l31 = lane & 31, lk = lane >> 5;
  const float sgn = g.conj_b ? -1.0f : 1.0f;

  f32x16 acc_r[NB][NB], acc_i[NB][NB];
#pragma unroll
  for (int i = 0; i < NB; ++i)
#pragma unroll
    for (int j = 0; j < NB; ++j) {
      acc_r[i][j] = f32x16{0};
      acc_i[i][j] = f32x16{0};
    }

  int kb = 0, ke = g.K;
  if (g.splits > 1) {
    kb = blockIdx.z * g.kchunk;
    ke = kb + g.kchunk < g.K ? kb + g.kchunk : g.K;
  }
  const int64_t bz = g.batch > 1 ? blockIdx.z : 0;
  const TIN* pa_r = reinterpret_cast<const TIN*>(g.a_r) + bz * g.a_bs;
  const TIN* pb_r = reinterpret_cast<const TIN*>(g.b_r) + bz * g.b_bs;
  const TIN* pa_i = CPLX ? reinterpret_cast<const TIN*>(g.a_i) + bz * g.a_bs : nullptr;
  const TIN* pb_i = CPLX ? reinterpret_cast<const TIN*>(g.b_i) + bz * g.b_bs : nullptr;
  TileRegs<NB> ra, rb, rai, rbi;
  auto fetch = [&](int k0) {
    ra = fetch_tile<TIN, NB>(pa_r, g.a_rs, g.a_cs, m0, k0, g.M, ke);
    rb = fetch_tile<TIN, NB>(pb_r, g.b_rs, g.b_cs, n0, k0, g.N, ke);
    if (CPLX) {
      rai = fetch_tile<TIN, NB>(pa_i, g.a_rs, g.a_cs, m0, k0, g.M, ke);
      rbi = fetch_tile<TIN, NB>(pb_i, g.b_rs, g.b_cs, n0, k0, g.N, ke);
    }
  };
  if (kb < ke) fetch(kb);
  int buf = 0;
  for (int k0 = kb; k0 < ke; k0 += GBK, buf ^= 1) {
    commit_tile<NB>(plane(buf, 0), ra, g.a_rs, g.a_cs);
    commit_tile<NB>(plane(buf, 1), rb, g.b_rs, g.b_cs);
    if (CPLX) {
      commit_tile<NB>(plane(buf, 2), rai, g.a_rs, g.a_cs);
      commit_tile<NB>(plane(buf, 3), rbi, g.b_rs, g.b_cs);
    }
    __syncthreads();
    if (k0 + GBK < ke) fetch(k0 + GBK);
    const float* Ar = plane(buf, 0);
    const float* Br = plane(buf, 1);
    const float* Ai = plane(buf, CPLX ? 2 : 0);
    const float* Bi = plane(buf, CPLX ? 3 : 1);
#pragma unroll
    for (int kk = 0; kk < GBK; kk += 2) {
      float ar[NB], br[NB], ai[NB], bi[NB];
#pragma unroll
      for (int i = 0; i < NB; ++i) {
        ar[i] = Ar[(kk + lk) * GLD + wm + i * 32 + l31];
        br[i] = Br[(kk + lk) * GLD + wn + i * 32 + l31];
        if (CPLX) {
          ai[i] = Ai[(kk + lk) * GLD + wm + i * 32 + l31];
          bi[i] = sgn * Bi[(kk + lk) * GLD + wn + i * 32 + l31];
        }
      }
#pragma unroll
      for (int i = 0; i < NB; ++i)
#pragma unroll
        for (int j = 0; j < NB; ++j) {
          acc_r[i][j] = __builtin_amdgcn_mfma_f32_32x32x2f32(ar[i], br[j], acc_r[i][j], 0, 0, 0);
          if (CPLX) {
            acc_r[i][j] = __builtin_amdgcn_mfma_f32_32x32x2f32(-ai[i], bi[j], acc_r[i][j], 0, 0, 0);
            acc_i[i][j] = __builtin_amdgcn_mfma_f32_32x32x2f32(ar[i], bi[j], acc_i[i][j], 0, 0, 0);
            acc_i[i][j] = __builtin_amdgcn_mfma_f32_32x32x2f32(ai[i], br[j], acc_i[i][j], 0, 0, 0);
          }
        }
    }
  }

  TOUT* cr = reinterpret_cast<TOUT*>(g.c_r) + bz * g.c_bs;
  TOUT* ci = reinterpret_cast<TOUT*>(g.c_i) + (CPLX ? bz * g.c_bs : 0);
  const float beta = gemm_beta(g);
  float* slab = g.splits > 1 ? reinterpret_cast<float*>(g.ws) + (int64_t)blockIdx.z * (CPLX ? 2 : 1) * g.M * g.N
                             : nullptr;
#pragma unroll
  for (int j = 0; j < NB; ++j) {
    const int col = n0 + wn + j * 32 + l31;
    if (col >= g.N) continue;
    const float b_r = g.bias_r ? g.bias_r[col] : 0.0f;
    const float b_i = (CPLX && g.bias_i) ? g.bias_i[col] : 0.0f;
#pragma unroll
    for (int i = 0; i < NB; ++i)
#pragma unroll
      for (int r = 0; r < 16; ++r) {
        const int row = m0 + wm + i * 32 + (r & 3) + 8 * (r >> 2) + 4 * lk;
        if (row >= g.M) continue;
        if (slab) {
          slab[(int64_t)row * g.N + col] = acc_r[i][j][r];
          if (CPLX) slab[(int64_t)g.M * g.N + (int64_t)row * g.N + col] = acc_i[i][j][r];
          continue;
        }
        const int64_t o = (int64_t)row * g.ldc + col;
        float vr = acc_r[i][j][r] + b_r;
        if (g.emul) vr *= gemm_emul(g, g.emul[o]);
        if (g.accumulate) vr += beta * io<TOUT>::ld(cr + o);
        io<TOUT>::st(cr + o, vr);
        if (CPLX) {
          float vi = acc_i[i][j][r] + b_i;
          if (g.emul && g.emul_both) vi *= gemm_emul(g, g.emul[o]);
          if (g.accumulate) vi += beta * io<TOUT>::ld(ci + o);
          io<TOUT>::st(ci + o, vi);
        }
      }
  }
}

static int gemm_generic_tile(int M, int N) {
  return (int64_t)((M + 127) / 128) * ((N + 127) / 128) <= 32 ? 64 : 128;
}

int gemm_generic_splits(int M, int N, int K) {
  const int bm = gemm_generic_tile(M, N);
  const int64_t tiles = (int64_t)((M + bm - 1) / bm) * ((N + bm - 1) / bm);
  const bool tiny = tiles <= 8;
  if (tiles >= 128 || K < (tiny ? 4 : 16) * GBK) return 1;
  int64_t s = 512 / tiles;
  const int64_t maxs = K / ((tiny ? 2 : 4) * GBK);
  if (s > maxs) s = maxs;
  if (s > 64) s = 64;
  return s < 2 ? 1 : (int)s;
}

int64_t gemm_generic_ws_bytes(int M, int N, int K, bool cplx) {
  const int s = gemm_generic_splits(M, N, K);
  return s > 1 ? (int64_t)s * (cplx ? 2 : 1) * M * N * (int64_t)sizeof(float) : 0;
}

template <typename TOUT>
__global__ __launch_bounds__(256) void generic_slab_reduce_kernel(const float* slabs, int splits,
                                                                  int64_t slab_stride, int M, int N,
                                                                  int64_t ldc, const float* bias_r, const float* bias_i,
                                                                  const float* emul, int emul_both, int emul_exp,
                                                                  int accumulate, const float* beta_p, TOUT* out_r,
                                                                  TOUT* out_i) {
  const int pl = blockIdx.y;
  const float* bias = pl ? bias_i : bias_r;
  TOUT* out = pl ? out_i : out_r;
  if (pl && !emul_both) emul = nullptr;
  slabs += (int64_t)pl * M * N;
  const float beta = (accumulate && beta_p) ? *beta_p : 1.0f;
  const int64_t n = (int64_t)M * N, stride = (int64_t)gridDim.x * 256;
  for (int64_t i = (int64_t)blockIdx.x * 256 + threadIdx.x; i < n; i += stride) {
    float a4[4] = {0.f, 0.f, 0.f, 0.f};
    int s = 0;
    for (; s + 3 < splits; s += 4) {
#pragma unroll
      for (int u = 0; u < 4; ++u) a4[u] += slabs[(int64_t)(s + u) * slab_stride + i];
    }
    for (; s < splits; ++s) a4[0] += slabs[(int64_t)s * slab_stride + i];
    float acc = (a4[0] + a4[1]) + (a4[2] + a4[3]);
    const int row = (int)(i / N), col = (int)(i - (int64_t)row * N);
    const int64_t o = (int64_t)row * ldc + col;
    if (bias) acc += bias[col];
    if (emul) acc *= emul_exp ? expf(emul[o]) : emul[o];
    if (accumulate) acc += beta * io<TOUT>::ld(out + o);
    io<TOUT>::st(out + o, acc);
  }
}

template <bool CPLX>
int launch_gemm_generic(const GemmArgs& g0, int in_dtype, int out_dtype, hipStream_t st) {
  if (g0.M <= 0 || g0.N <= 0) return 0;
  GemmArgs g = g0;
  g.splits = 1;
  const int want = g.batch > 1 ? 1 : gemm_generic_splits(g.M, g.N, g.K);
  if (want > 1 && g.ws && g.ws_bytes >= gemm_generic_ws_bytes(g.M, g.N, g.K, CPLX)) {
    g.splits = want;
    g.kchunk = (((g.K + GBK - 1) / GBK + want - 1) / want) * GBK;
  }
  if (g.batch > 65535) return CPLXAMD_ESHAPE;
  const int bm = gemm_generic_tile(g.M, g.N);
  dim3 grid((g.N + bm - 1) / bm, (g.M + bm - 1) / bm, g.batch > 1 ? g.batch : g.splits);
  const int smem = 2 * (CPLX ? 4 : 2) * (bm == 64 ? GT<1>::PLANE : GT<2>::PLANE) * (int)sizeof(float);
  auto go = [&](auto kern) -> int {
    if (smem > 64 * 1024) {
      hipError_t e = hipFuncSetAttribute((const void*)kern, hipFuncAttributeMaxDynamicSharedMemorySize, smem);
      if (e != hipSuccess) return (int)e;
    }
    kern<<<grid, 256, smem, st>>>(g);
    CPLXAMD_CHECK_LAUNCH();
    return 0;
  };
  int rc;
#define GEN_GO(TI, TO) (bm == 64 ? go(gemm_generic_kernel<TI, TO, CPLX, 1>) : go(gemm_generic_kernel<TI, TO, CPLX, 2>))
  if (in_dtype == CPLXAMD_F32 && out_dtype == CPLXAMD_F32) rc = GEN_GO(float, float);
  else if (in_dtype == CPLXAMD_BF16 && out_dtype == CPLXAMD_F32) rc = GEN_GO(bf16_t, float);
  else if (in_dtype == CPLXAMD_BF16 && out_dtype == CPLXAMD_BF16) rc = GEN_GO(bf16_t, bf16_t);
  else if (in_dtype == CPLXAMD_F32 && out_dtype == CPLXAMD_BF16) rc = GEN_GO(float, bf16_t);
  else return CPLXAMD_EINVAL;
#undef GEN_GO
  if (rc) return rc;
  if (g.splits > 1) {
    const int64_t slab = (int64_t)g.M * g.N, stride = (CPLX ? 2 : 1) * slab;
    const dim3 rgrid(stream_grid(slab, 256), CPLX ? 2 : 1);
    const float* src = (const float*)g.ws;
    if (out_dtype == CPLXAMD_F32)
      generic_slab_reduce_kernel<float><<<rgrid, 256, 0, st>>>(src, g.splits, stride, g.M, g.N, g.ldc, g.bias_r, g.bias_i,
                                                              g.emul, g.emul_both, g.emul_exp, g.accumulate, g.beta,
                                                              (float*)g.c_r, (float*)g.c_i);
    else
      generic_slab_reduce_kernel<bf16_t><<<rgrid, 256, 0, st>>>(src, g.splits, stride, g.M, g.N, g.ldc, g.bias_r, g.bias_i,
                                                               g.emul, g.emul_both, g.emul_exp, g.accumulate, g.beta,
                                                               (bf16_t*)g.c_r, (bf16_t*)g.c_i);
    CPLXAMD_CHECK_LAUNCH();
  }
  return 0;
}

template int launch_gemm_generic<true>(const GemmArgs&, int, int, hipStream_t);
template int launch_gemm_generic<false>(const GemmArgs&, int, int, hipStream_t);

}
```

Measured before the change: 2.427 million samples/s.

## Prefetch epilogue operands during final K tiles in w4 GEMM kernel

During the last K-loop tiles, the main-loop buffer loads are redirected through masked base, offset and num_records selection to prefetch epilogue operands (emul, accumulate source, or fused grad/x planes) into the staging registers. The epilogue then consumes those operands with a software-pipelined request/operand scheme, and a separate fused bf16 epilogue is added. With beta==0 the accumulate reads use zero num_records, and gemm_cin treats those values as zero, so the old C is never actually fetched. The aim is to hide the epilogue's global-load latency behind the final MMA work, at the cost of higher register pressure and considerable complexity.

```diff
diff --git a/cplxmodule_amd/csrc/gemm.h b/cplxmodule_amd/csrc/gemm.h
--- a/cplxmodule_amd/csrc/gemm.h
+++ b/cplxmodule_amd/csrc/gemm.h
@@ -24,6 +24,7 @@
 };
 
 __device__ __forceinline__ float gemm_beta(const GemmArgs& g) { return (g.accumulate && g.beta) ? *g.beta : 1.0f; }
+__device__ __forceinline__ float gemm_cin(float beta, float c) { return beta == 0.0f ? 0.0f : c; }
 __device__ __forceinline__ float gemm_alpha(const GemmArgs& g) { return g.scale_a ? g.scale_a[1] * g.scale_b[1] : 1.0f; }
 __device__ __forceinline__ float gemm_alpha_inv(const GemmArgs& g) { return g.scale_a ? g.scale_a[0] * g.scale_b[0] : 1.0f; }
 
diff --git a/cplxmodule_amd/csrc/gemm_bf16_impl.h b/cplxmodule_amd/csrc/gemm_bf16_impl.h
--- a/cplxmodule_amd/csrc/gemm_bf16_impl.h
+++ b/cplxmodule_amd/csrc/gemm_bf16_impl.h
@@ -480,7 +480,7 @@
                 if (g.accumulate) {
                   const f4 p = ld4(out + o);
 #pragma unroll
-                  for (int e = 0; e < 4; ++e) v.v[e] += beta * p.v[e];
+                  for (int e = 0; e < 4; ++e) v.v[e] += beta * gemm_cin(beta, p.v[e]);
                 }
                 nt_store16(out + o, v);
               } else {
@@ -489,7 +489,7 @@
                   if (col + e < g.N) {
                     float x = v.v[e];
                     if (g.emul && (!pl || g.emul_both)) x *= gemm_emul(g, g.emul[o + e]);
-                    if (g.accumulate) x += beta * out[o + e];
+                    if (g.accumulate) x += beta * gemm_cin(beta, out[o + e]);
                     out[o + e] = x;
                   }
               }
@@ -572,11 +572,11 @@
           if (g.accumulate) {
             const f4 p = ld4(cr + o);
 #pragma unroll
-            for (int e = 0; e < 4; ++e) vr.v[e] += beta * p.v[e];
+            for (int e = 0; e < 4; ++e) vr.v[e] += beta * gemm_cin(beta, p.v[e]);
             if (CPLX) {
               const f4 p2 = ld4(ci + o);
 #pragma unroll
-              for (int e = 0; e < 4; ++e) vi.v[e] += beta * p2.v[e];
+              for (int e = 0; e < 4; ++e) vi.v[e] += beta * gemm_cin(beta, p2.v[e]);
             }
           }
           st4(cr + o, vr);
@@ -587,12 +587,12 @@
             if (col + e >= g.N) break;
             float xr = vr.v[e] + ((g.bias_r && !bias_in_acc) ? g.bias_r[col + e] : 0.f);
             if (g.emul) xr *= gemm_emul(g, g.emul[o + e]);
-            if (g.accumulate) xr += beta * io<TOUT>::ld(cr + o + e);
+            if (g.accumulate) xr += beta * gemm_cin(beta, io<TOUT>::ld(cr + o + e));
             io<TOUT>::st(cr + o + e, xr);
             if (CPLX) {
               float xi = vi.v[e] + ((g.bias_i && !bias_in_acc) ? g.bias_i[col + e] : 0.f);
               if (g.emul && g.emul_both) xi *= gemm_emul(g, g.emul[o + e]);
-              if (g.accumulate) xi += beta * io<TOUT>::ld(ci + o + e);
+              if (g.accumulate) xi += beta * gemm_cin(beta, io<TOUT>::ld(ci + o + e));
               io<TOUT>::st(ci + o + e, xi);
             }
           }
@@ -769,7 +769,7 @@
     if (accumulate) {
       const f4 o = ld4(out + 4 * i);
 #pragma unroll
-      for (int e = 0; e < 4; ++e) acc.v[e] += beta * o.v[e];
+      for (int e = 0; e < 4; ++e) acc.v[e] += beta * gemm_cin(beta, o.v[e]);
     }
     st4(out + 4 * i, acc);
   }
diff --git a/cplxmodule_amd/csrc/gemm_bf16_w4.hip b/cplxmodule_amd/csrc/gemm_bf16_w4.hip
--- a/cplxmodule_amd/csrc/gemm_bf16_w4.hip
+++ b/cplxmodule_amd/csrc/gemm_bf16_w4.hip
@@ -117,6 +117,10 @@
   const int wm = (wid / C::WN) * (32 * IB), wn = (wid % C::WN) * (32 * JB);
   const int l31 = lane & 31, lk = lane >> 5;
   const int l15 = lane & 15, lg = (lane >> 4) & 1;
+  const int wid_s = __builtin_amdgcn_readfirstlane(tid >> 6);
+  auto lane_id = []() __attribute__((always_inline)) {
+    return (int)__builtin_amdgcn_mbcnt_hi(~0u, __builtin_amdgcn_mbcnt_lo(~0u, 0u));
+  };
 
   const int64_t lda = TA ? g.a_cs : g.a_rs, ldb = TB ? g.b_cs : g.b_rs;
   const int64_t ka = TA ? lda * 2 : 2, kb = TB ? ldb * 2 : 2;
@@ -155,6 +159,8 @@
 
   f32x16 acc_r[IB][JB], acc_i[CPLX ? IB : 1][JB];
 
+  const float beta = gemm_beta(g);
+  const uint32_t nrec_acc = beta == 0.0f ? 0u : 0x7ffffffeu;
   const bool has_bias = g.bias_r != nullptr;
   f4 bias_v[NPL][JB][4];
   if (has_bias) {
@@ -182,7 +188,45 @@
   }
 
   u32x4 st[2][NL];
-  auto load_piece = [&](auto PAR, auto Q, int kt) __attribute__((always_inline)) {
+  bool epre = false;
+  uint32_t emask = 0;
+  const char* eb[3] = {nullptr, nullptr, nullptr};
+  uint32_t evo = 0, eps = 0;
+  bool enop2 = false;
+  uint32_t enr[2] = {0x7ffffffeu, 0x7ffffffeu};
+  auto epi_has_ops = [&]() __attribute__((always_inline)) {
+    if constexpr (PERSIST) return false;
+    else if constexpr (sizeof(TOUT) == 2) return g.fga != nullptr;
+    else return g.emul != nullptr || g.accumulate != 0;
+  };
+  auto epi_setup = [&](bool last) __attribute__((always_inline)) {
+    if constexpr (!PERSIST) {
+      epre = last && epi_has_ops();
+      emask = epre ? ~0u : 0u;
+      const int lane = lane_id();
+      const int wm = (wid_s / C::WN) * (32 * IB), wn = (wid_s % C::WN) * (32 * JB);
+      if constexpr (sizeof(TOUT) == 2) {
+        const int64_t off = ((int64_t)m0 * g.fld + n0) * 2;
+        eb[0] = (const char*)g.fga + off;
+        eb[1] = (const char*)g.fx_r + off;
+        eb[2] = (const char*)(CPLX ? g.fx_i : g.fx_r) + off;
+        evo = (uint32_t)((((int64_t)(wm + (lane >> 3)) * g.fld + wn + (lane & 7) * 8)) * 2);
+        eps = (uint32_t)__builtin_amdgcn_readfirstlane((int)(uint32_t)(8 * g.fld * 2));
+      } else {
+        const int64_t off = ((int64_t)m0 * g.ldc + n0) * 4;
+        const char* em = (const char*)g.emul + off;
+        const char* ec = (const char*)g.c_r + off;
+        enop2 = g.emul != nullptr && g.accumulate != 0;
+        eb[0] = g.emul ? em : ec;
+        eb[1] = (g.emul && !g.accumulate) ? em : ec;
+        enr[0] = g.emul ? 0x7ffffffeu : nrec_acc;
+        enr[1] = (g.emul && !g.accumulate) ? 0x7ffffffeu : nrec_acc;
+        evo = (uint32_t)((((int64_t)(wm + (lane >> 4)) * g.ldc + wn + (lane & 15) * 4)) * 4);
+        eps = (uint32_t)__builtin_amdgcn_readfirstlane((int)(uint32_t)(4 * g.ldc * 4));
+      }
+    }
+  };
+  auto load_piece = [&](auto PAR, auto Q, int kt, auto EPIQ) __attribute__((always_inline)) {
     constexpr int par = decltype(PAR)::value, q = decltype(Q)::value;
     constexpr int pl = q / (PA + PB), r = q % (PA + PB);
     constexpr bool isa = r < PA;
@@ -194,9 +238,22 @@
       const int64_t kby = (int64_t)(kt & ~1) * BK * (isa ? ka : kb);
       base = (isa ? pa[pl] : pb[pl]) + kby;
     }
-    __amdgpu_buffer_rsrc_t rs = __builtin_amdgcn_make_buffer_rsrc((void*)base, 0, 0x7ffffffe, 0x00020000);
-    const uint32_t so = (uint32_t)j * (isa ? psa : psb) + (par ? (isa ? qa : qb) : 0u);
-    const uint32_t vo = (isa ? voa : vob) + ((par && !(isa ? TA : TB)) ? 64u : 0u);
+    uint32_t so = (uint32_t)j * (isa ? psa : psb) + (par ? (isa ? qa : qb) : 0u);
+    uint32_t vo = (isa ? voa : vob) + ((par && !(isa ? TA : TB)) ? 64u : 0u);
+    uint32_t nrec = 0x7ffffffeu;
+    if constexpr (decltype(EPIQ)::value && !PERSIST) {
+      constexpr int n = 2 * q + par;
+      constexpr int NOP16 = NPL + 1;
+      const char* ebase;
+      uint32_t eso;
+      if constexpr (sizeof(TOUT) == 2) { ebase = eb[n % NOP16]; eso = (uint32_t)(n / NOP16) * eps; }
+      else { ebase = eb[n & 1]; eso = (enop2 ? (uint32_t)(n >> 1) : (uint32_t)n) * eps; nrec = (nrec & ~emask) | (enr[n & 1] & emask); }
+      const uint64_t m64 = ((uint64_t)emask << 32) | emask;
+      base = (const char*)(((uintptr_t)base & ~m64) | ((uintptr_t)ebase & m64));
+      so = (so & ~emask) | (eso & emask);
+      vo = (vo & ~emask) | (evo & emask);
+    }
+    __amdgpu_buffer_rsrc_t rs = __builtin_amdgcn_make_buffer_rsrc((void*)base, 0, (int)nrec, 0x00020000);
     st[par][q] = __builtin_amdgcn_raw_buffer_load_b128(rs, vo, so, 0);
   };
   const uint32_t smem_off = (uint32_t)(uintptr_t)smem;
@@ -286,7 +343,7 @@
   const int klen = g.splits > 1 ? ((g.K - kbase) < g.kchunk ? (g.K - kbase) : g.kchunk) : g.K;
   const int nt = __builtin_amdgcn_readfirstlane(klen / BK);
 
-  auto sub = [&](auto F, auto PAR, auto H, auto RS, auto RKS, auto WS, int kt_next) __attribute__((always_inline)) {
+  auto sub = [&](auto F, auto PAR, auto H, auto RS, auto RKS, auto WS, int kt_next, auto EPIQ) __attribute__((always_inline)) {
     constexpr int f = decltype(F)::value, par = decltype(PAR)::value, h = decltype(H)::value;
     using I_F = std::integral_constant<int, f>;
     using I_G = std::integral_constant<int, 1 - f>;
@@ -314,8 +371,8 @@
         using PIECE = std::integral_constant<int, h * NW + wi>;
         write_piece(I_P{}, PIECE{}, WS);
         if constexpr (par == 1) {
-          W4_SB(); load_piece(I0_{}, PIECE{}, kt_next);
-          W4_SB(); load_piece(I1_{}, PIECE{}, kt_next);
+          W4_SB(); load_piece(I0_{}, PIECE{}, kt_next, EPIQ);
+          W4_SB(); load_piece(I1_{}, PIECE{}, kt_next, EPIQ);
         }
       }
     };
@@ -349,7 +406,7 @@
     plane_bases(mn, nn, pan, pbn);
   };
   if constexpr (PERSIST) { look_ahead(); set_request(0, std::false_type{}); }
-  for_pieces([&](auto Q) __attribute__((always_inline)) { load_piece(I0{}, Q, 0); load_piece(I1{}, Q, 0); });
+  for_pieces([&](auto Q) __attribute__((always_inline)) { load_piece(I0{}, Q, 0, std::false_type{}); load_piece(I1{}, Q, 0, std::false_type{}); });
 #pragma unroll
   for (int i = 0; i < IB; ++i)
 #pragma unroll
@@ -368,7 +425,7 @@
   {
     const int kt = nt > 2 ? 2 : nt - 2;
     if constexpr (PERSIST) set_request(kt, std::true_type{});
-    for_pieces([&](auto Q) __attribute__((always_inline)) { load_piece(I0{}, Q, kt); load_piece(I1{}, Q, kt); });
+    for_pieces([&](auto Q) __attribute__((always_inline)) { load_piece(I0{}, Q, kt, std::false_type{}); load_piece(I1{}, Q, kt, std::false_type{}); });
   }
   asm volatile("s_waitcnt lgkmcnt(0)" ::: "memory");
   __builtin_amdgcn_s_barrier();
@@ -386,7 +443,7 @@
   };
   first_frags();
 
-  auto tile = [&](auto SS, auto PP, int t, auto REDIR) __attribute__((always_inline)) {
+  auto tile = [&](auto SS, auto PP, int t, auto REDIR, auto EPIQ) __attribute__((always_inline)) {
     constexpr int s = decltype(SS)::value, par = decltype(PP)::value;
     using CUR = std::integral_constant<int, s>; using NXT = std::integral_constant<int, (s + 1) % 3>;
     using WR = std::integral_constant<int, (s + 2) % 3>;
@@ -396,11 +453,11 @@
       ktn = t + ahead;
       if constexpr (par == 1) set_request(ktn, REDIR);
     }
-    sub(I0{}, PP, I0{}, CUR{}, I1{}, WR{}, ktn);
+    sub(I0{}, PP, I0{}, CUR{}, I1{}, WR{}, ktn, EPIQ);
     asm volatile("s_waitcnt lgkmcnt(1)" ::: "memory");
     __builtin_amdgcn_s_barrier();
     W4_SB();
-    sub(I1{}, PP, I1{}, NXT{}, I0{}, WR{}, ktn);
+    sub(I1{}, PP, I1{}, NXT{}, I0{}, WR{}, ktn, EPIQ);
   };
   auto rotate = [&](auto R) __attribute__((always_inline)) {
     constexpr int r = decltype(R)::value;
@@ -418,21 +475,24 @@
   {
     int t = 0;
     using RD = std::true_type;
+    using NQ = std::false_type; using EQ = std::true_type;
     for (; t + 6 <= nt; t += 6) {
-      tile(I0{}, I0{}, t, RD{});
-      tile(I1{}, I1{}, t + 1, RD{});
-      tile(I2{}, I0{}, t + 2, RD{});
-      tile(I0{}, I1{}, t + 3, RD{});
-      tile(I1{}, I0{}, t + 4, RD{});
-      tile(I2{}, I1{}, t + 5, RD{});
+      tile(I0{}, I0{}, t, RD{}, NQ{});
+      tile(I1{}, I1{}, t + 1, RD{}, NQ{});
+      tile(I2{}, I0{}, t + 2, RD{}, NQ{});
+      tile(I0{}, I1{}, t + 3, RD{}, NQ{});
+      tile(I1{}, I0{}, t + 4, RD{}, NQ{});
+      tile(I2{}, I1{}, t + 5, RD{}, NQ{});
     }
     if (t < nt) {
-      tile(I0{}, I0{}, t, RD{});
-      tile(I1{}, I1{}, t + 1, RD{});
+      tile(I0{}, I0{}, t, RD{}, NQ{});
+      epi_setup(t + 2 >= nt);
+      tile(I1{}, I1{}, t + 1, RD{}, EQ{});
       t += 2;
       if (t < nt) {
-        tile(I2{}, I0{}, t, RD{});
-        tile(I0{}, I1{}, t + 1, RD{});
+        tile(I2{}, I0{}, t, RD{}, NQ{});
+        epi_setup(true);
+        tile(I0{}, I1{}, t + 1, RD{}, EQ{});
         if constexpr (PERSIST) rotate(I1{});
       } else {
         if constexpr (PERSIST) rotate(I2{});
@@ -462,7 +522,6 @@
     float* base = reinterpret_cast<float*>(g.ws) + (int64_t)split * NPL * slab;
     out_r = base; out_i = base + slab;
   }
-  const float beta = gemm_beta(g);
   asm volatile("s_waitcnt lgkmcnt(0)" ::: "memory");
   if constexpr (!PERSIST) __builtin_amdgcn_s_barrier();
   auto tile_rsrc = [&](const void* plane, int64_t ld, int esize) __attribute__((always_inline)) {
@@ -476,34 +535,17 @@
     __builtin_amdgcn_raw_buffer_store_b128(v, r, vo, so, 0);
   };
   if constexpr (sizeof(TOUT) == 2) {
-    auto epi16 = [&](auto FUSE) __attribute__((always_inline)) {
-      constexpr bool fuse = decltype(FUSE)::value;
+    auto epi16 = [&]() __attribute__((always_inline)) {
       constexpr int PITCH = 144;
-      const int tid_e = PERSIST ? (int)opaque((uint32_t)tid) : tid;
+      const int tid_e = PERSIST ? (int)opaque((uint32_t)tid) : wid_s * 64 + lane_id();
       const int lane = tid_e & 63, wid = tid_e >> 6;
       const int wm = (wid / C::WN) * (32 * IB), wn = (wid % C::WN) * (32 * JB);
       const int l31 = lane & 31, lk = lane >> 5;
       const uint32_t vo_c = (uint32_t)((((int64_t)(wm + (lane >> 3)) * g.ldc + wn + (lane & 7) * 8)) * 2);
       char* reg = smem + (PERSIST ? (CPLX ? sl[2] : (uint32_t)C::SMEM) : 0u) + wid * (64 * PITCH);
-      const uint32_t vo_f = fuse ? (uint32_t)((((int64_t)(wm + (lane >> 3)) * g.fld + wn + (lane & 7) * 8)) * 2) : 0u;
       const uint32_t p8c = (uint32_t)__builtin_amdgcn_readfirstlane((int)(uint32_t)(8 * g.ldc * 2));
-      const uint32_t p8f = (uint32_t)__builtin_amdgcn_readfirstlane((int)(uint32_t)(8 * g.fld * 2));
-      const __amdgpu_buffer_rsrc_t rga = tile_rsrc(fuse ? g.fga : g.c_r, fuse ? g.fld : g.ldc, 2);
       const __amdgpu_buffer_rsrc_t rout0 = tile_rsrc(out_r, g.ldc, 2), rout1 = tile_rsrc(CPLX ? out_i : out_r, g.ldc, 2);
-      const __amdgpu_buffer_rsrc_t rx0 = tile_rsrc(fuse ? g.fx_r : g.c_r, fuse ? g.fld : g.ldc, 2);
-      const __amdgpu_buffer_rsrc_t rx1 = tile_rsrc(fuse ? (CPLX ? g.fx_i : g.fx_r) : g.c_r, fuse ? g.fld : g.ldc, 2);
       constexpr int NR = NPL * (JB / 2) * (IB / 2);
-      u32x4 gv[2][fuse ? 8 : 1], xv[2][fuse ? 8 : 1];
-      auto load_ops = [&](int r) __attribute__((always_inline)) {
-        const int pl = r / ((JB / 2) * (IB / 2)), jh = (r / (IB / 2)) % (JB / 2), ih = r % (IB / 2);
-#pragma unroll
-        for (int pass = 0; pass < 8; ++pass) {
-          const uint32_t so = (uint32_t)(ih * 8 + pass) * p8f + (uint32_t)(jh * 128);
-          gv[r & 1][pass] = ldb128(rga, vo_f, so);
-          xv[r & 1][pass] = ldb128(pl ? rx1 : rx0, vo_f, so);
-        }
-      };
-      if constexpr (fuse) load_ops(0);
       if constexpr (PERSIST) W4_VMCNT(0);
 #pragma unroll
       for (int r = 0; r < NR; ++r) {
@@ -526,56 +568,151 @@
               if constexpr (PERSIST) W4_SB();
             }
         asm volatile("s_waitcnt lgkmcnt(0)" ::: "memory");
-        if constexpr (fuse) {
-          if (r + 1 < NR) { W4_SB(); load_ops(r + 1); W4_SB(); }
-        }
 #pragma unroll
         for (int pass = 0; pass < 8; ++pass) {
           const int rl = pass * 8 + (lane >> 3), c8 = (lane & 7) * 8;
           const u32x4 v = *reinterpret_cast<const u32x4*>(reg + rl * PITCH + c8 * 2);
           const uint32_t so = (uint32_t)(ih * 8 + pass) * p8c + (uint32_t)(jh * 128);
-          if constexpr (fuse) {
-            u32x4 ow;
-#pragma unroll
-            for (int e = 0; e < 4; ++e) {
-              const float d0 = __uint_as_float(v[e] << 16), d1 = __uint_as_float(v[e] & 0xffff0000u);
-              const float x0 = __uint_as_float(xv[r & 1][pass][e] << 16), x1 = __uint_as_float(xv[r & 1][pass][e] & 0xffff0000u);
-              const float g0 = __uint_as_float(gv[r & 1][pass][e] << 16), g1 = __uint_as_float(gv[r & 1][pass][e] & 0xffff0000u);
-              ow[e] = pack_bf16(fmaf(2.0f * x0, g0, d0), fmaf(2.0f * x1, g1, d1));
-            }
-            stb128(ow, rout, vo_c, so);
-          } else {
-            stb128(v, rout, vo_c, so);
-          }
+          stb128(v, rout, vo_c, so);
         }
         asm volatile("s_waitcnt lgkmcnt(0)" ::: "memory");
         if constexpr (PERSIST) W4_VMCNT(16);
         W4_SB();
       }
     };
-    if constexpr (PERSIST) epi16(std::false_type{});
-    else { if (g.fga) epi16(std::true_type{}); else epi16(std::false_type{}); }
+    auto epi16f = [&]() __attribute__((always_inline)) {
+      constexpr int PITCH = 144;
+      constexpr int PLANE = 64 * PITCH;
+      constexpr int NOP = NPL + 1;
+      constexpr int NR = (JB / 2) * (IB / 2);
+      static_assert(8 * NOP == 2 * NL, "one round of operands fills the staging registers");
+      const int lane = lane_id(), wid = wid_s;
+      const int wm = (wid / C::WN) * (32 * IB), wn = (wid % C::WN) * (32 * JB);
+      const int l31 = lane & 31, lk = lane >> 5;
+      const uint32_t vo_c = (uint32_t)((((int64_t)(wm + (lane >> 3)) * g.ldc + wn + (lane & 7) * 8)) * 2);
+      char* reg = smem + wid * (NPL * PLANE);
+      const uint32_t p8c = (uint32_t)__builtin_amdgcn_readfirstlane((int)(uint32_t)(8 * g.ldc * 2));
+      const __amdgpu_buffer_rsrc_t rout0 = tile_rsrc(out_r, g.ldc, 2), rout1 = tile_rsrc(CPLX ? out_i : out_r, g.ldc, 2);
+      const bool pre = epre;
+      epi_setup(false);
+      auto request = [&](int n, int r) __attribute__((always_inline)) {
+        const int jh = r / (IB / 2), ih = r % (IB / 2);
+        const __amdgpu_buffer_rsrc_t rs = __builtin_amdgcn_make_buffer_rsrc((void*)eb[n % NOP], 0, 0x7ffffffe, 0x00020000);
+        st[n & 1][n >> 1] = ldb128(rs, evo, (uint32_t)(ih * 8 + n / NOP) * eps + (uint32_t)(jh * 128));
+      };
+      if (!pre) {
+#pragma unroll
+        for (int n = 0; n < 8 * NOP; ++n) request(n, 0);
+      }
+#pragma unroll
+      for (int r = 0; r < NR; ++r) {
+        const int jh = r / (IB / 2), ih = r % (IB / 2);
+#pragma unroll
+        for (int pl = 0; pl < NPL; ++pl)
+#pragma unroll
+          for (int ii = 0; ii < 2; ++ii)
+#pragma unroll
+            for (int jj = 0; jj < 2; ++jj)
+#pragma unroll
+              for (int q = 0; q < 4; ++q) {
+                const int cl = jj * 32 + 8 * q + 4 * lk;
+                f4 v;
+#pragma unroll
+                for (int e = 0; e < 4; ++e)
+                  v.v[e] = pl ? acc_i[CPLX ? ih * 2 + ii : 0][jh * 2 + jj][4 * q + e] : acc_r[ih * 2 + ii][jh * 2 + jj][4 * q + e];
+                st4(reinterpret_cast<bf16_t*>(reg + pl * PLANE + (ii * 32 + l31) * PITCH + cl * 2), v);
+              }
+        asm volatile("s_waitcnt lgkmcnt(0)" ::: "memory");
+        u32x4 dnext[NPL];
+#pragma unroll
+        for (int pl = 0; pl < NPL; ++pl) dnext[pl] = *reinterpret_cast<const u32x4*>(reg + pl * PLANE + (lane >> 3) * PITCH + (lane & 7) * 16);
+#pragma unroll
+        for (int pass = 0; pass < 8; ++pass) {
+          const int rl = pass * 8 + (lane >> 3), c8 = (lane & 7) * 8;
+          const uint32_t so = (uint32_t)(ih * 8 + pass) * p8c + (uint32_t)(jh * 128);
+          u32x4 d[NPL];
+#pragma unroll
+          for (int pl = 0; pl < NPL; ++pl) d[pl] = dnext[pl];
+          if (pass + 1 < 8) {
+#pragma unroll
+            for (int pl = 0; pl < NPL; ++pl) dnext[pl] = *reinterpret_cast<const u32x4*>(reg + pl * PLANE + (rl + 8) * PITCH + c8 * 2);
+            W4_SB();
+          }
+          const u32x4 gw = st[(pass * NOP) & 1][(pass * NOP) >> 1];
+          float g0[4], g1[4];
+#pragma unroll
+          for (int e = 0; e < 4; ++e) { g0[e] = __uint_as_float(gw[e] << 16); g1[e] = __uint_as_float(gw[e] & 0xffff0000u); }
+          u32x4 ow[NPL];
+#pragma unroll
+          for (int pl = 0; pl < NPL; ++pl) {
+            const u32x4 xw = st[(pass * NOP + 1 + pl) & 1][(pass * NOP + 1 + pl) >> 1];
+#pragma unroll
+            for (int e = 0; e < 4; ++e) {
+              const float d0 = __uint_as_float(d[pl][e] << 16), d1 = __uint_as_float(d[pl][e] & 0xffff0000u);
+              const float x0 = __uint_as_float(xw[e] << 16), x1 = __uint_as_float(xw[e] & 0xffff0000u);
+              ow[pl][e] = pack_bf16(fmaf(2.0f * x0, g0[e], d0), fmaf(2.0f * x1, g1[e], d1));
+            }
+          }
+          if (r + 1 < NR) {
+            W4_SB();
+#pragma unroll
+            for (int o = 0; o < NOP; ++o) request(pass * NOP + o, r + 1);
+            W4_SB();
+          }
+#pragma unroll
+          for (int pl = 0; pl < NPL; ++pl) stb128(ow[pl], pl ? rout1 : rout0, vo_c, so);
+        }
+        asm volatile("s_waitcnt lgkmcnt(0)" ::: "memory");
+        W4_SB();
+      }
+    };
+    if constexpr (PERSIST) epi16();
+    else { if (g.fga) epi16f(); else epi16(); }
   } else {
     auto epi32 = [&](auto HM, auto HACC) __attribute__((always_inline)) {
-      constexpr bool hm = decltype(HM)::value, hacc = decltype(HACC)::value;
+      constexpr bool hm = decltype(HM)::value != 0, hexp = decltype(HM)::value == 2, hacc = decltype(HACC)::value;
       constexpr int PITCH = 272;
+      const int lane = lane_id(), wid = wid_s;
+      const int wm = (wid / C::WN) * (32 * IB), wn = (wid % C::WN) * (32 * JB);
+      const int l31 = lane & 31, lk = lane >> 5;
       char* reg = smem + wid * (32 * PITCH);
       const uint32_t vo = (uint32_t)((((int64_t)(wm + (lane >> 4)) * g.ldc + wn + (lane & 15) * 4)) * 4);
       const uint32_t p4 = (uint32_t)__builtin_amdgcn_readfirstlane((int)(uint32_t)(4 * g.ldc * 4));
       const __amdgpu_buffer_rsrc_t rm = tile_rsrc(hm ? (const void*)g.emul : g.c_r, g.ldc, 4);
       const __amdgpu_buffer_rsrc_t rout0 = tile_rsrc(out_r, g.ldc, 4), rout1 = tile_rsrc(CPLX ? out_i : out_r, g.ldc, 4);
       constexpr int NR = NPL * (JB / 2) * IB;
-      u32x4 mv[2][hm ? 8 : 1], pv[2][hacc ? 8 : 1];
-      auto load_ops = [&](int r) __attribute__((always_inline)) {
+      constexpr int NOP = (hm ? 1 : 0) + (hacc ? 1 : 0);
+      constexpr int D = 4 / (NOP ? NOP : 4);
+      constexpr int NST = 2 * NL;
+      u32x4 ex[NOP ? 32 - NST : 1];
+      auto acc_rsrc = [&](const void* plane) __attribute__((always_inline)) {
+        const char* base = (const char*)plane + ((int64_t)m0 * g.ldc + n0) * 4;
+        return __builtin_amdgcn_make_buffer_rsrc((void*)base, 0, (int)nrec_acc, 0x00020000);
+      };
+      const __amdgpu_buffer_rsrc_t racc0 = acc_rsrc(out_r), racc1 = acc_rsrc(CPLX ? out_i : out_r);
+      const bool pre = epre;
+      epi_setup(false);
+      auto request = [&](int r, int pass, int o) __attribute__((always_inline)) {
         const int pl = r / ((JB / 2) * IB), jh = (r / IB) % (JB / 2), i = r % IB;
-#pragma unroll
-        for (int pass = 0; pass < 8; ++pass) {
-          const uint32_t so = (uint32_t)(i * 8 + pass) * p4 + (uint32_t)(jh * 256);
-          if constexpr (hm) mv[r & 1][pass] = ldb128(rm, vo, so);
-          if constexpr (hacc) pv[r & 1][pass] = ldb128(pl ? rout1 : rout0, vo, so);
+        const uint32_t so = (uint32_t)(i * 8 + pass) * p4 + (uint32_t)(jh * 256);
+        const int n = ((r % D) * 8 + pass) * NOP + o;
+        const u32x4 w = ldb128((hm && o == 0) ? rm : (pl ? racc1 : racc0), vo, so);
+        if (n < NST) st[n & 1][(n < NST ? n : 0) >> 1] = w; else ex[n < NST ? 0 : n - NST] = w;
+      };
+      auto operand = [&](int r, int pass, int o) __attribute__((always_inline)) -> u32x4 {
+        const int n = ((r % D) * 8 + pass) * NOP + o;
+        return n < NST ? st[n & 1][(n < NST ? n : 0) >> 1] : ex[n < NST ? 0 : n - NST];
+      };
+      if constexpr (NOP > 0) {
+        if (!pre) {
+#pragma unroll
+          for (int n = 0; n < NST; ++n)
+            if (n / (8 * NOP) < NR) request(n / (8 * NOP), (n / NOP) % 8, n % NOP);
         }
-      };
-      if constexpr (hm || hacc) load_ops(0);
+#pragma unroll
+        for (int n = NST; n < 32; ++n)
+          if (n / (8 * NOP) < NR) request(n / (8 * NOP), (n / NOP) % 8, n % NOP);
+      }
 #pragma unroll
       for (int r = 0; r < NR; ++r) {
         const int pl = r / ((JB / 2) * IB), jh = (r / IB) % (JB / 2), i = r % IB;
@@ -592,34 +729,56 @@
             st4(reinterpret_cast<float*>(reg + l31 * PITCH + cl * 4), v);
           }
         asm volatile("s_waitcnt lgkmcnt(0)" ::: "memory");
-        if constexpr (hm || hacc) {
-          if (r + 1 < NR) { W4_SB(); load_ops(r + 1); W4_SB(); }
-        }
+        auto staged = [&](int pass) __attribute__((always_inline)) {
+          return ld4(reinterpret_cast<const float*>(reg + (pass * 4 + (lane >> 4)) * PITCH + (lane & 15) * 16));
+        };
+        f4 vnext = staged(0);
 #pragma unroll
         for (int pass = 0; pass < 8; ++pass) {
-          const int rl = pass * 4 + (lane >> 4), c4 = (lane & 15) * 4;
-          f4 v = ld4(reinterpret_cast<const float*>(reg + rl * PITCH + c4 * 4));
+          f4 v = vnext;
+          if constexpr (NOP > 0) {
+            if (pass + 1 < 8) { vnext = staged(pass + 1); W4_SB(); }
+          } else {
+            if (pass > 0) v = staged(pass);
+          }
+          float mul[4] = {1.f, 1.f, 1.f, 1.f};
+          if constexpr (hm) {
+            const u32x4 mw = operand(r, pass, 0);
+#pragma unroll
+            for (int e = 0; e < 4; ++e) mul[e] = hexp ? expf(__uint_as_float(mw[e])) : __uint_as_float(mw[e]);
+          }
           const uint32_t so = (uint32_t)(i * 8 + pass) * p4 + (uint32_t)(jh * 256);
           if constexpr (hm) {
 #pragma unroll
             for (int e = 0; e < 4; ++e) {
-              v.v[e] *= gemm_emul(g, __uint_as_float(mv[r & 1][pass][e]));
+              v.v[e] *= mul[e];
               asm volatile("" : "+v"(v.v[e]));
             }
           }
           if constexpr (hacc) {
-#pragma unroll
-            for (int e = 0; e < 4; ++e) v.v[e] += beta * __uint_as_float(pv[r & 1][pass][e]);
+            const u32x4 pw = operand(r, pass, NOP - 1);
+#pragma unroll
+            for (int e = 0; e < 4; ++e) v.v[e] += beta * __uint_as_float(pw[e]);
           }
           const u32x4 w = {__float_as_uint(v.v[0]), __float_as_uint(v.v[1]), __float_as_uint(v.v[2]), __float_as_uint(v.v[3])};
+          if constexpr (NOP > 0) {
+            if (r + D < NR) {
+              W4_SB();
+#pragma unroll
+              for (int o = 0; o < NOP; ++o) request(r + D, pass, o);
+              W4_SB();
+            }
+          }
           stb128(w, rout, vo, so);
         }
         asm volatile("s_waitcnt lgkmcnt(0)" ::: "memory");
         W4_SB();
       }
     };
-    if (g.emul) { if (g.accumulate) epi32(std::true_type{}, std::true_type{}); else epi32(std::true_type{}, std::false_type{}); }
-    else { if (g.accumulate) epi32(std::false_type{}, std::true_type{}); else epi32(std::false_type{}, std::false_type{}); }
+    using M0 = std::integral_constant<int, 0>; using M1 = std::integral_constant<int, 1>; using M2 = std::integral_constant<int, 2>;
+    if (g.emul && g.emul_exp) { if (g.accumulate) epi32(M2{}, std::true_type{}); else epi32(M2{}, std::false_type{}); }
+    else if (g.emul) { if (g.accumulate) epi32(M1{}, std::true_type{}); else epi32(M1{}, std::false_type{}); }
+    else { if (g.accumulate) epi32(M0{}, std::true_type{}); else epi32(M0{}, std::false_type{}); }
   }
   if constexpr (!PERSIST) {
     break;
@@ -642,7 +801,7 @@
     first_frags();
     if constexpr (CPLX) {
       set_request(2, std::false_type{});
-      for_pieces([&](auto Q) __attribute__((always_inline)) { load_piece(I0{}, Q, 2); load_piece(I1{}, Q, 2); });
+      for_pieces([&](auto Q) __attribute__((always_inline)) { load_piece(I0{}, Q, 2, std::false_type{}); load_piece(I1{}, Q, 2, std::false_type{}); });
     }
     if constexpr (!CPLX) W4_VMCNT(0);
   }
diff --git a/cplxmodule_amd/csrc/gemm_generic.hip b/cplxmodule_amd/csrc/gemm_generic.hip
--- a/cplxmodule_amd/csrc/gemm_generic.hip
+++ b/cplxmodule_amd/csrc/gemm_generic.hip
@@ -162,12 +162,12 @@
         const int64_t o = (int64_t)row * g.ldc + col;
         float vr = acc_r[i][j][r] + b_r;
         if (g.emul) vr *= gemm_emul(g, g.emul[o]);
-        if (g.accumulate) vr += beta * io<TOUT>::ld(cr + o);
+        if (g.accumulate) vr += beta * gemm_cin(beta, io<TOUT>::ld(cr + o));
         io<TOUT>::st(cr + o, vr);
         if (CPLX) {
           float vi = acc_i[i][j][r] + b_i;
           if (g.emul && g.emul_both) vi *= gemm_emul(g, g.emul[o]);
-          if (g.accumulate) vi += beta * io<TOUT>::ld(ci + o);
+          if (g.accumulate) vi += beta * gemm_cin(beta, io<TOUT>::ld(ci + o));
           io<TOUT>::st(ci + o, vi);
         }
       }
@@ -222,7 +222,7 @@
     const int64_t o = (int64_t)row * ldc + col;
     if (bias) acc += bias[col];
     if (emul) acc *= emul_exp ? expf(emul[o]) : emul[o];
-    if (accumulate) acc += beta * io<TOUT>::ld(out + o);
+    if (accumulate) acc += beta * gemm_cin(beta, io<TOUT>::ld(out + o));
     io<TOUT>::st(out + o, acc);
   }
 }
```

Result: no change. 2.431 million samples/s (median of 2 runs) (+0.2%).
